# compbio-UofT/shrimp

Measured on AMD Instinct MI355X. Metric: reads/sec mapped (whole node), 100bp LS reads vs 3Gbp ref, 1/2/4/8 GPUs, higher is better.
Workload: dtype int16

## Files before the change

shrimp_amd/csrc/gm_common.h:

```cpp
#pragma once
#include <hip/hip_runtime.h>
#include <stdint.h>
#include <string>
#include <vector>
#include "../../include/gmapper_hip.h"

#define GM_MAX_SEEDS 16
#define GM_WAVE 64

void gm_set_error(const char* fmt, ...);
#define GM_HIP(call)                                                                          \
  do {                                                                                        \
    hipError_t e_ = (call);                                                                   \
    if (e_ != hipSuccess) {                                                                   \
      gm_set_error("%s failed: %s (%s:%d)", #call, hipGetErrorString(e_), __FILE__, __LINE__); \
      return GM_E_NODEVICE;                                                                   \
    }                                                                                         \
  } while (0)

struct GmSeedDev {
  uint64_t mask;
  int span, weight;
  const uint32_t* dir;
  const uint32_t* pos;
  const uint32_t* bkt;
  const uint32_t* sdir;
  const uint32_t* spos;
  uint32_t n_pos;
};

#define GM_MP_CAP 8192
#define GM_MP_FLAG 0x80000000u
struct GmMpDev {
  int mode;
  int dmin[2], dmax[2];
  int mate_dmin[2], mate_dmax[2];
  uint32_t* rows; const uint32_t* cnt;
  uint32_t* out_rows; uint32_t* out_cnt;
};
__device__ __forceinline__ bool gm_mp_reach(const uint32_t* row, uint32_t n, long long lo, long long hi, uint32_t* first = nullptr) {
  if (hi < 0 || n == 0) return false;
  if (lo < 0) lo = 0;
  uint32_t a = 0, z = n;
  while (a < z) { const uint32_t m = (a + z) >> 1; if ((long long)(row[m] & ~GM_MP_FLAG) < lo) a = m + 1; else z = m; }
  if (first) *first = a;
  return a < n && (long long)(row[a] & ~GM_MP_FLAG) <= hi;
}

struct GmIndexDev {
  const uint32_t* genome;
  const uint32_t* genome_cs;
  int colour;
  int hflag;
  int cs_flip;
  int no_region_counts;
  GmMpDev mp;
  const uint8_t* contig_rna;
  int genome_is_rna;
  const uint8_t* read_rna;
  uint64_t total_len;
  int n_contigs;
  const uint32_t* contig_off;
  int n_seeds, min_seed_span, max_seed_span;
  int slab_bits, n_slabs;
  int region_bits, region_overlap;
  uint32_t list_cutoff;
  GmSeedDev seed[GM_MAX_SEEDS];
};

struct GmScoreDev {
  int match, mismatch;
  int a_go, a_ge, b_go, b_ge;
  int anchor_width;
  int match_mode, min_matches;
  int skip_strands;
  int num_tmp_outputs;
  int tiebreak_rev;
  int hash_filter_calls;
  int gapless;
  int local;
  double wgen_thr_frac;
  double vect_thr_frac, full_thr_frac;
  int wgen_abs, vect_abs, full_abs;
};

struct GmHit {
  uint32_t g_off;
  int32_t  ax, ay;
  int32_t  alen, awidth;
  int32_t  score_window_gen;
  int32_t  score_vector;
  int32_t  pct_score_vector;
  uint16_t cn, w_len;
  uint16_t matches, flags;
};

#define GM_MAX_OPS 2048
struct GmFullRes {
  int32_t read_idx;
  int16_t st, gen_st;
  uint32_t cn; uint32_t g_off;
  int32_t w_len;
  int32_t score_vector;
  int32_t score_max, matches, score_window_gen;
  int32_t score;
  int32_t read_start, rmapped, genome_start, gmapped;
  int32_t n_match, n_mismatch, n_ins, n_del;
  int32_t n_ops; uint32_t ops_off;
  int32_t sort_idx;
  uint32_t hit_slot;
  int32_t n_xover;
};

__host__ __device__ __forceinline__ uint64_t gm_cmpl_tab(bool rna) { return 0xFBCDE56879A00123ull + (rna ? 1ull : 0ull); }

#ifdef GM_NO_READ_RNA
#define GM_READ_RNA(ix, rd) false
#else
#define GM_READ_RNA(ix, rd) ((ix).read_rna && (ix).read_rna[rd])
#endif
#define GM_SEAM_RNA 0x100

__device__ __forceinline__ uint32_t gm_read_code(const uint32_t* __restrict__ rw, int read_len, int st, int colour, int i, bool rna = false) {
  if (colour) {
    if (st && i == 0) return 15u;
    const int src = st ? (read_len - i) : i;
    return (rw[src >> 3] >> ((src & 7) * 4)) & 0xf;
  }
  const int src = st ? (read_len - 1 - i) : i;
  uint32_t c = (rw[src >> 3] >> ((src & 7) * 4)) & 0xf;
  if (st) { const uint64_t cm = gm_cmpl_tab(rna); c = (uint32_t)(cm >> (c * 4)) & 0xf; }
  return c;
}

#define GM_HASH_TABLE_POWER 12
__host__ __device__ __forceinline__ uint32_t gm_hash32(uint32_t a) {
  a = (a + 0x7ed55d16u) + (a << 12); a = (a ^ 0xc761c23cu) ^ (a >> 19); a = (a + 0x165667b1u) + (a << 5);
  a = (a + 0xd3a2646cu) ^ (a << 9); a = (a + 0xfd7046c5u) + (a << 3); a = (a ^ 0xb55a4f09u) ^ (a >> 16);
  return a;
}
__device__ __forceinline__ uint32_t gm_mapidx(const GmIndexDev& ix, uint64_t mask, int span, const uint8_t* kmer) {
  uint32_t mapidx = 0;
  if (!ix.hflag) {
    for (int t = 0; t < span; t++) if ((mask >> t) & 1) mapidx = (mapidx << 2) | (kmer[span - 1 - t] & 3u);
    return mapidx;
  }
  const int nw = (ix.max_seed_span + 7) >> 3;
  for (int w = 0; w < nw; w++) {
    uint32_t word = 0;
    for (int t = 0; t < 8; t++) { const int age = 8 * w + t; if (age < span && ((mask >> age) & 1)) word |= (uint32_t)(kmer[span - 1 - age] & 0xfu) << (4 * t); }
    mapidx = gm_hash32(word ^ mapidx);
  }
  return mapidx & ((1u << (2 * GM_HASH_TABLE_POWER)) - 1u);
}

static inline int gm_ceil_div(long long a, long long b) { return (int)((a + b - 1) / b); }
```

shrimp_amd/csrc/gm_host.hip:

```cpp
#include <algorithm>
#include <atomic>
#include <chrono>
#include <cmath>
#include <cstdarg>
#include <cstddef>
#include <cstdio>
#include <cstdlib>
#include <cstring>
#include <memory>
#include <thread>
#include <mutex>
#include <condition_variable>
#include <deque>
#include <functional>
#include <future>
#include <map>
#include <unordered_map>
#include <zlib.h>
#include "gm_common.h"
#include "gm_internal.h"

static thread_local char g_err[512] = "";
void gm_set_error(const char* fmt, ...) {
  va_list ap; va_start(ap, fmt); vsnprintf(g_err, sizeof g_err, fmt, ap); va_end(ap);
}
extern "C" const char* gm_last_error(void) { return g_err; }
extern "C" int gm_device_count(void) { int n = 0; if (hipGetDeviceCount(&n) != hipSuccess) return 0; return n; }
hipError_t gm_lds_at_least(const void* kernel, size_t bytes) {
  if (bytes <= 48 * 1024) return hipSuccess;
  int dev = 0; hipError_t e = hipGetDevice(&dev);
  if (e != hipSuccess) return e;
  static std::mutex m; static std::map<std::pair<int, const void*>, size_t> raised;
  std::lock_guard<std::mutex> lk(m);
  size_t& cur = raised[{dev, kernel}];
  if (bytes <= cur) return hipSuccess;
  e = hipFuncSetAttribute(kernel, hipFuncAttributeMaxDynamicSharedMemorySize, (int)bytes);
  if (e == hipSuccess) cur = bytes;
  return e;
}
static struct { std::mutex m; char* p = nullptr; size_t cap = 0; char* live = nullptr; size_t live_cap = 0; } g_outcache;
static char* outcache_take(size_t want, size_t* cap) {
  std::lock_guard<std::mutex> g(g_outcache.m);
  if (g_outcache.p && g_outcache.cap >= want) { char* r = g_outcache.p; *cap = g_outcache.cap; g_outcache.p = nullptr; g_outcache.cap = 0; return r; }
  return nullptr;
}
static void outcache_track(char* p, size_t cap) { std::lock_guard<std::mutex> g(g_outcache.m); g_outcache.live = p; g_outcache.live_cap = cap; }
static void gm_text_pool_drop();
extern "C" void gm_release_cache(void) { { std::lock_guard<std::mutex> g(g_outcache.m); free(g_outcache.p); g_outcache.p = nullptr; g_outcache.cap = 0; } gm_text_pool_drop(); }
extern "C" void gm_free(void* p) {
  if (!p) return;
  { std::lock_guard<std::mutex> g(g_outcache.m);
    if (p == g_outcache.live && g_outcache.live_cap >= ((size_t)16 << 20)) {
      g_outcache.live = nullptr;
      if (g_outcache.p && g_outcache.cap >= g_outcache.live_cap) {  }
      else { free(g_outcache.p); g_outcache.p = (char*)p; g_outcache.cap = g_outcache.live_cap; return; }
    } else if (p == g_outcache.live) g_outcache.live = nullptr;
  }
  free(p);
}

extern "C" void gm_params_default(gm_params_t* p) {
  memset(p, 0, sizeof *p);
  p->match_score = 10; p->mismatch_score = -15;
  p->a_gap_open_score = -33; p->a_gap_extend_score = -7; p->b_gap_open_score = -33; p->b_gap_extend_score = -3;
  p->window_len = 140.0; p->window_overlap = 90.0; p->window_gen_threshold = 55.0;
  p->sw_vect_threshold = 50.0; p->sw_full_threshold = 50.0;
  p->match_mode = 2; p->num_outputs = 10; p->num_tmp_outputs = 30; p->anchor_width = 8;
  p->region_bits = 11; p->region_overlap = 50; p->list_cutoff = 0; p->hash_filter_calls = 1; p->tiebreak_rev = 1;
  p->sam_unaligned = 0; p->longest_read_len = 1000; p->strata = 0; p->max_alignments = 0;
  p->colour_space = 0; p->crossover_score = -20; p->indel_taboo_len = 0; p->pr_xover = 0.03; p->local_alignment = 0; p->ungapped = 0; p->hash_seeds = 0; p->output_format = 0; p->print_read_seq = 0; p->strand_only = 0;
  p->single_best_mapping = 0; p->all_contigs = 0; p->no_mapping_qualities = 0; p->no_improper_mappings = 0;
  p->extra_sam_fields = 0; p->sam_r2 = 0; memset(p->read_group, 0, sizeof p->read_group);
  p->trim_front = 0; p->trim_end = 0; p->trim_first = 1; p->trim_second = 1; p->trim_illumina = 0; p->min_avg_qv = 10; p->ignore_qvs = 0; p->no_qv_check = 0;
}
extern "C" int gm_abi_sizeof(int which) {
  switch (which) { case 0: return (int)sizeof(gm_params_t); case 1: return (int)sizeof(gm_pair_opts_t); case 2: return (int)sizeof(gm_map_stats_t); case 3: return (int)sizeof(gm_merge_options_t); }
  return -1;
}
static inline bool gm_mqv_on(const gm_params_t& P) { return !P.local_alignment && !P.no_mapping_qualities; }
extern "C" void gm_params_default_cs(gm_params_t* p) {
  gm_params_default(p);
  p->colour_space = 1; p->mismatch_score = -24; p->sw_vect_threshold = 47.0; p->sw_full_threshold = 50.0;
}

static GmScoreDev make_score(const gm_params_t& P) {
  GmScoreDev s; memset(&s, 0, sizeof s);
  s.match = P.match_score;
  s.mismatch = P.colour_space ? P.match_score + P.crossover_score : P.mismatch_score;
  s.a_go = -P.a_gap_open_score; s.a_ge = -P.a_gap_extend_score; s.b_go = -P.b_gap_open_score; s.b_ge = -P.b_gap_extend_score;
  s.anchor_width = P.anchor_width; s.match_mode = P.match_mode; s.min_matches = P.match_mode;
  s.skip_strands = P.strand_only == 1 ? 2 : (P.strand_only == 2 ? 1 : 0);
  s.num_tmp_outputs = P.num_tmp_outputs; s.tiebreak_rev = P.tiebreak_rev; s.hash_filter_calls = P.hash_filter_calls; s.local = P.local_alignment ? 1 : 0; s.gapless = P.ungapped ? 1 : 0;
  auto frac = [](double thr, double* f, int* a) { if (thr < 0) { *f = -1.0; *a = (int)(-thr); } else { *f = thr / 100.0; *a = 0; } };
  frac(P.window_gen_threshold, &s.wgen_thr_frac, &s.wgen_abs);
  frac(P.sw_vect_threshold, &s.vect_thr_frac, &s.vect_abs);
  frac(P.sw_full_threshold, &s.full_thr_frac, &s.full_abs);
  return s;
}

GmIndexDev GmIndexHost::dev_view() const {
  GmIndexDev d; memset(&d, 0, sizeof d);
  d.genome = d_genome; d.genome_cs = d_genome_cs; d.colour = params.colour_space ? 1 : 0; d.hflag = params.hash_seeds ? 1 : 0; d.total_len = total_len; d.n_contigs = n_contigs; d.contig_off = d_contig_off;
  d.contig_rna = d_contig_rna; d.genome_is_rna = genome_is_rna; d.read_rna = nullptr;
  d.n_seeds = n_seeds; d.min_seed_span = min_seed_span; d.max_seed_span = max_seed_span;
  d.slab_bits = slab_bits; d.n_slabs = n_slabs; d.region_bits = params.region_bits; d.region_overlap = params.region_overlap;
  d.list_cutoff = list_cutoff;
  for (int i = 0; i < n_seeds; i++) {
    d.seed[i].mask = seeds[i].mask; d.seed[i].span = seeds[i].span; d.seed[i].weight = seeds[i].weight;
    d.seed[i].dir = seeds[i].d_dir; d.seed[i].pos = seeds[i].d_pos; d.seed[i].bkt = seeds[i].d_bkt; d.seed[i].n_pos = seeds[i].n_pos;
    d.seed[i].sdir = strips_ready ? seeds[i].d_sdir : nullptr; d.seed[i].spos = strips_ready ? seeds[i].d_spos : nullptr;
  }
  return d;
}

static int add_seed(GmIndexHost* ix, const char* s) {
  if (ix->n_seeds >= GM_MAX_SEEDS) return GM_E_ARG;
  GmSeedHost& sd = ix->seeds[ix->n_seeds];
  sd.mask = 0; sd.span = (int)strlen(s); sd.weight = 0; sd.text = s;
  if (sd.span < 1 || sd.span > 32) return GM_E_ARG;
  for (int i = 0; i < sd.span; i++) {
    if (s[i] != '0' && s[i] != '1') return GM_E_ARG;
    sd.mask = (sd.mask << 1) | (uint64_t)(s[i] == '1'); sd.weight += (s[i] == '1');
  }
  if (sd.weight < 1 || (!ix->params.hash_seeds && sd.weight > 14)) return GM_E_ARG;
  sd.kbits = ix->params.hash_seeds ? 2 * GM_HASH_TABLE_POWER : 2 * sd.weight;
  ix->max_seed_span = std::max(ix->max_seed_span, sd.span);
  ix->min_seed_span = std::min(ix->min_seed_span, sd.span);
  ix->n_seeds++;
  return GM_OK;
}

static void choose_slabs(GmIndexHost* ix) {
  int bits = 12;
  while ((1ull << bits) < ix->total_len) bits++;
  int sb = std::min(bits, 29);
  if (const char* e = gm_tune("GM_SLAB_BITS")) sb = std::max(ix->params.region_bits + 2, std::min(31, atoi(e)));
  ix->slab_bits = sb;
  ix->n_slabs = (int)((ix->total_len + (1ull << sb) - 1) >> sb);
  if (ix->n_slabs < 1) ix->n_slabs = 1;
}

static int index_tables(gm_index* ix, int n_contigs, const uint32_t* contig_len, const char* const* contig_names) {
  ix->n_contigs = n_contigs;
  ix->contig_off.resize(n_contigs + 1);
  uint64_t tot = 0;
  for (int c = 0; c < n_contigs; c++) {
    ix->contig_off[c] = (uint32_t)tot; tot += contig_len[c];
    char nm[64]; snprintf(nm, sizeof nm, "contig%d", c + 1);
    ix->names.push_back(contig_names && contig_names[c] ? contig_names[c] : nm);
  }
  if (tot >= (1ull << 32)) { gm_set_error("genome of %llu bp exceeds the reference's 32-bit global coordinates", (unsigned long long)tot); return GM_E_ARG; }
  ix->contig_off[n_contigs] = (uint32_t)tot;
  ix->total_len = tot;
  if (ix->params.list_cutoff == 0) {
    int maxw = 0; for (int i = 0; i < ix->n_seeds; i++) maxw = std::max(maxw, ix->seeds[i].weight);
    if (ix->params.hash_seeds) maxw = GM_HASH_TABLE_POWER;
    uint32_t cutoff = 1000; unsigned long long p4 = 1ull << (2 * maxw);
    if ((uint32_t)((100ull * tot) / p4) > cutoff) cutoff = (uint32_t)((100ull * tot) / p4);
    ix->list_cutoff = cutoff;
  } else ix->list_cutoff = ix->params.list_cutoff;
  choose_slabs(ix);
  ix->genome_words = (tot + 7) / 8 + 64;
  GM_HIP(hipMalloc(&ix->d_contig_off, (size_t)(n_contigs + 1) * 4));
  GM_HIP(hipMemcpy(ix->d_contig_off, ix->contig_off.data(), (size_t)(n_contigs + 1) * 4, hipMemcpyHostToDevice));
  return GM_OK;
}
static int index_prepare(gm_index* ix, int n_contigs, const uint32_t* const* contigs, const uint32_t* contig_len, const char* const* contig_names) {
  { const int rc = index_tables(ix, n_contigs, contig_len, contig_names); if (rc != GM_OK) return rc; }
  std::vector<uint32_t> g(ix->genome_words, 0);
  for (int c = 0; c < n_contigs; c++) {
    const uint64_t off = ix->contig_off[c]; const uint32_t* src = contigs[c]; const uint64_t len = contig_len[c];
    const int sh = (int)(off & 7) * 4; uint64_t w0 = off >> 3; const uint64_t nw = (len + 7) / 8;
    for (uint64_t k = 0; k < nw; k++) {
      uint32_t w = src[k];
      if (k == nw - 1 && (len & 7)) w &= (1u << ((len & 7) * 4)) - 1u;
      g[w0 + k] |= w << sh;
      if (sh) g[w0 + k + 1] |= w >> (32 - sh);
    }
  }
  GM_HIP(hipMalloc(&ix->d_genome, ix->genome_words * 4));
  GM_HIP(hipMemcpy(ix->d_genome, g.data(), ix->genome_words * 4, hipMemcpyHostToDevice));
  return GM_OK;
}

extern "C" void gm_index_free(gm_index_t* ix);
static int index_seeds(gm_index* ix, int n_seeds, const char* const* seeds) {
  int rc = GM_OK;
  if (n_seeds == 0) {
    rc |= add_seed(ix, "11110111101111"); rc |= add_seed(ix, "1111011100100001111"); rc |= add_seed(ix, "1111000011001101111");
  } else for (int i = 0; i < n_seeds; i++) rc |= add_seed(ix, seeds[i]);
  return rc;
}
extern "C" int gm_index_build(gm_index_t** out, int device, int n_contigs, const uint32_t* const* contigs,
                              const uint32_t* contig_len, const char* const* contig_names,
                              int n_seeds, const char* const* seeds, const gm_params_t* params) {
  if (!out || n_contigs < 1 || !contigs || !contig_len) { gm_set_error("gm_index_build: bad arguments"); return GM_E_ARG; }
  if (gm_device_count() <= device) { gm_set_error("no HIP device %d (the seed index lives in HBM; there is no CPU path)", device); return GM_E_NODEVICE; }
  GM_HIP(hipSetDevice(device));
  gm_index* ix = new gm_index();
  ix->device = device;
  if (params) ix->params = *params; else gm_params_default(&ix->params);
  int rc = index_seeds(ix, n_seeds, seeds);
  if (rc != GM_OK) { delete ix; gm_set_error("invalid spaced seed"); return GM_E_ARG; }
  rc = index_prepare(ix, n_contigs, contigs, contig_len, contig_names);
  if (rc != GM_OK) { gm_index_free(ix); return rc; }
  hipStream_t stream; GM_HIP(hipStreamCreate(&stream));
  rc = gm_index_build_device(ix, stream);
  (void)hipStreamDestroy(stream);
  if (rc != GM_OK) { gm_index_free(ix); return rc; }
  *out = ix;
  return GM_OK;
}

extern "C" int gm_index_build_fasta(gm_index_t** out, int device, int n_files, const char* const* paths,
                                    int n_seeds, const char* const* seeds, const gm_params_t* params) {
  if (!out || n_files < 1 || !paths) { gm_set_error("gm_index_build_fasta: bad arguments"); return GM_E_ARG; }
  if (gm_device_count() <= device) { gm_set_error("no HIP device %d (the seed index lives in HBM; there is no CPU path)", device); return GM_E_NODEVICE; }
  GM_HIP(hipSetDevice(device));
  const auto t0 = std::chrono::steady_clock::now();
  gm_index* ix = new gm_index();
  ix->device = device;
  if (params) ix->params = *params; else gm_params_default(&ix->params);
  int rc = index_seeds(ix, n_seeds, seeds);
  if (rc != GM_OK) { delete ix; gm_set_error("invalid spaced seed"); return GM_E_ARG; }
  GmFastaGenome G;
  rc = gm_fasta_to_device(n_files, paths, &G);
  if (rc != GM_OK) { delete ix; return rc; }
  ix->d_genome = G.d_genome;
  std::vector<const char*> nptr(G.names.size());
  for (size_t c = 0; c < G.names.size(); c++) nptr[c] = G.names[c].c_str();
  rc = index_tables(ix, (int)G.lens.size(), G.lens.data(), nptr.data());
  if (rc == GM_OK && (ix->total_len != G.total || ix->genome_words != G.words)) { gm_set_error("gm_index_build_fasta: contig lengths do not add up to the bases packed"); rc = GM_E_ARG; }
  if (rc != GM_OK) { gm_index_free(ix); return rc; }
  const auto t1 = std::chrono::steady_clock::now();
  hipStream_t stream = nullptr;
  if (hipStreamCreate(&stream) != hipSuccess) { gm_index_free(ix); gm_set_error("hipStreamCreate failed"); return GM_E_NODEVICE; }
  rc = gm_index_build_device(ix, stream);
  (void)hipStreamDestroy(stream);
  if (rc != GM_OK) { gm_index_free(ix); return rc; }
  ix->fasta_to_bitfield_s = std::chrono::duration<double>(t1 - t0).count();
  ix->fasta_total_s = std::chrono::duration<double>(std::chrono::steady_clock::now() - t0).count();
  *out = ix;
  return GM_OK;
}
extern "C" int gm_index_n_contigs(const gm_index_t* ix) { return ix ? ix->n_contigs : GM_E_ARG; }
extern "C" int gm_index_contig(const gm_index_t* ix, int c, const char** name, uint32_t* len) {
  if (!ix || c < 0 || c >= ix->n_contigs) { gm_set_error("gm_index_contig: no contig %d", c); return GM_E_ARG; }
  if (name) *name = ix->names[c].c_str();
  if (len) *len = ix->contig_off[c + 1] - ix->contig_off[c];
  return GM_OK;
}
extern "C" int gm_sam_header(const gm_index_t* ix, const char* rg_id, const char* rg_sample, const char* command_line, char** text, size_t* len) {
  if (!ix || !text || !len) { gm_set_error("gm_sam_header: bad arguments"); return GM_E_ARG; }
  std::string h = "@HD\tVN:1.0\tSO:unsorted\n";
  for (int c = 0; c < ix->n_contigs; c++) h += "@SQ\tSN:" + ix->names[c] + "\tLN:" + std::to_string(ix->contig_off[c + 1] - ix->contig_off[c]) + "\n";
  if (rg_id) h += std::string("@RG\tID:") + rg_id + "\tSM:" + (rg_sample ? rg_sample : "") + "\n";
  if (command_line) h += std::string("@PG\tID:gmapper\tVN:2.2.3\tCL:") + command_line + "\n";
  char* p = (char*)malloc(h.size() + 1);
  if (!p) return GM_E_NOMEM;
  memcpy(p, h.c_str(), h.size() + 1);
  *text = p; *len = h.size();
  return GM_OK;
}
extern "C" int gm_index_build_timing(const gm_index_t* ix, double* to_bitfield_s, double* total_s) {
  if (!ix || ix->fasta_total_s <= 0) { gm_set_error("gm_index_build_timing: not an index built by gm_index_build_fasta"); return GM_E_ARG; }
  if (to_bitfield_s) *to_bitfield_s = ix->fasta_to_bitfield_s;
  if (total_s) *total_s = ix->fasta_total_s;
  return GM_OK;
}

extern "C" void gm_index_free(gm_index_t* ix) {
  if (!ix) return;
  (void)hipSetDevice(ix->device);
  (void)hipFree(ix->d_genome); (void)hipFree(ix->d_genome_cs); (void)hipFree(ix->d_contig_off); (void)hipFree(ix->d_contig_rna);
  for (int i = 0; i < ix->n_seeds; i++) { (void)hipFree(ix->seeds[i].d_dir); (void)hipFree(ix->seeds[i].d_pos); (void)hipFree(ix->seeds[i].d_bkt);
                                           (void)hipFree(ix->seeds[i].d_sdir); (void)hipFree(ix->seeds[i].d_spos); }
  delete ix;
}
extern "C" uint32_t gm_index_list_cutoff(const gm_index_t* ix) { return ix->list_cutoff; }
extern "C" int gm_index_n_slabs(const gm_index_t* ix) { return ix->n_slabs; }
extern "C" int gm_index_has_buckets(const gm_index_t* ix) { return ix->seeds[0].d_bkt != nullptr; }
extern "C" uint64_t gm_index_bytes(const gm_index_t* ix) {
  uint64_t b = ix->genome_words * 4 * (ix->d_genome_cs ? 2 : 1);
  for (int i = 0; i < ix->n_seeds; i++) b += (ix->seeds[i].dir_words + (uint64_t)ix->seeds[i].n_pos + (ix->seeds[i].d_bkt ? (16ull << ix->seeds[i].kbits) : 0ull) +
                                            (ix->seeds[i].d_sdir ? (1ull << ix->seeds[i].kbits) + 1 + ix->seeds[i].n_spos : 0ull)) * 4;
  return b;
}
extern "C" int gm_index_get_list(const gm_index_t* ix, int sn, uint32_t mapidx, uint32_t* len, uint32_t* positions, uint32_t cap) {
  if (sn < 0 || sn >= ix->n_seeds || mapidx >= (1u << ix->seeds[sn].kbits)) return GM_E_ARG;
  GM_HIP(hipSetDevice(ix->device));
  uint32_t be[2];
  GM_HIP(hipMemcpy(&be[0], ix->seeds[sn].d_dir + (size_t)mapidx * ix->n_slabs, 4, hipMemcpyDeviceToHost));
  GM_HIP(hipMemcpy(&be[1], ix->seeds[sn].d_dir + (size_t)(mapidx + 1) * ix->n_slabs, 4, hipMemcpyDeviceToHost));
  *len = be[1] - be[0];
  uint32_t n = std::min(*len, cap);
  if (n && positions) GM_HIP(hipMemcpy(positions, ix->seeds[sn].d_pos + be[0], (size_t)n * 4, hipMemcpyDeviceToHost));
  return GM_OK;
}
extern "C" int gm_index_device_array(const gm_index_t* ix, int kind, void** dev_ptr, uint64_t* bytes) {
  if (kind == 0) { *dev_ptr = ix->d_genome; *bytes = ix->genome_words * 4; return GM_OK; }
  if (kind == 1 + 3 * ix->n_seeds) { *dev_ptr = ix->d_genome_cs; *bytes = ix->d_genome_cs ? ix->genome_words * 4 : 0; return GM_OK; }
  const int sn = (kind - 1) / 3, what = (kind - 1) % 3; if (kind < 0 || sn < 0 || sn >= ix->n_seeds) return GM_E_ARG;
  if (what == 0) { *dev_ptr = ix->seeds[sn].d_dir; *bytes = (ix->seeds[sn].dir_words + 16) * 4; }
  else if (what == 1) { *dev_ptr = ix->seeds[sn].d_pos; *bytes = ((uint64_t)ix->seeds[sn].n_pos + 64) * 4; }
  else { *dev_ptr = ix->seeds[sn].d_bkt; *bytes = ix->seeds[sn].d_bkt ? (16ull << ix->seeds[sn].kbits) * 4 : 0; }
  return GM_OK;
}

struct MetaHdr { uint64_t magic, total_len, genome_words; int32_t n_contigs, n_seeds, slab_bits, n_slabs; uint32_t list_cutoff, pad; gm_params_t params;
                 uint32_t n_pos[GM_MAX_SEEDS]; uint64_t dir_words[GM_MAX_SEEDS]; uint32_t has_bkt[GM_MAX_SEEDS]; };
extern "C" int gm_index_meta(const gm_index_t* ix, void* meta, uint64_t* meta_bytes) {
  std::string blob;
  MetaHdr h; memset(&h, 0, sizeof h);
  h.magic = 0x474D4958ull; h.total_len = ix->total_len; h.genome_words = ix->genome_words; h.n_contigs = ix->n_contigs; h.n_seeds = ix->n_seeds;
  h.slab_bits = ix->slab_bits; h.n_slabs = ix->n_slabs; h.list_cutoff = ix->list_cutoff; h.params = ix->params;
  for (int i = 0; i < ix->n_seeds; i++) { h.n_pos[i] = ix->seeds[i].n_pos; h.dir_words[i] = ix->seeds[i].dir_words; h.has_bkt[i] = ix->seeds[i].d_bkt != nullptr; }
  blob.append((const char*)&h, sizeof h);
  blob.append((const char*)ix->contig_off.data(), (size_t)(ix->n_contigs + 1) * 4);
  for (auto& n : ix->names) { blob += n; blob.push_back('\0'); }
  for (int i = 0; i < ix->n_seeds; i++) { blob += ix->seeds[i].text; blob.push_back('\0'); }
  if (meta && *meta_bytes >= blob.size()) memcpy(meta, blob.data(), blob.size());
  *meta_bytes = blob.size();
  return GM_OK;
}
extern "C" int gm_index_alloc_like(gm_index_t** out, int device, const void* meta, uint64_t meta_bytes) {
  if (meta_bytes < sizeof(MetaHdr)) return GM_E_ARG;
  MetaHdr h; memcpy(&h, meta, sizeof h);
  if (h.magic != 0x474D4958ull) return GM_E_ARG;
  if (gm_device_count() <= device) { gm_set_error("no HIP device %d", device); return GM_E_NODEVICE; }
  GM_HIP(hipSetDevice(device));
  gm_index* ix = new gm_index();
  ix->device = device; ix->params = h.params; ix->total_len = h.total_len; ix->genome_words = h.genome_words; ix->n_contigs = h.n_contigs;
  ix->slab_bits = h.slab_bits; ix->n_slabs = h.n_slabs; ix->list_cutoff = h.list_cutoff;
  const char* p = (const char*)meta + sizeof h;
  ix->contig_off.assign((const uint32_t*)p, (const uint32_t*)p + h.n_contigs + 1); p += (size_t)(h.n_contigs + 1) * 4;
  for (int c = 0; c < h.n_contigs; c++) { ix->names.push_back(p); p += strlen(p) + 1; }
  for (int i = 0; i < h.n_seeds; i++) { if (add_seed(ix, p) != GM_OK) { delete ix; return GM_E_ARG; } p += strlen(p) + 1; }
  GM_HIP(hipMalloc(&ix->d_genome, ix->genome_words * 4));
  if (ix->params.colour_space) GM_HIP(hipMalloc(&ix->d_genome_cs, ix->genome_words * 4));
  GM_HIP(hipMalloc(&ix->d_contig_off, (size_t)(h.n_contigs + 1) * 4));
  GM_HIP(hipMemcpy(ix->d_contig_off, ix->contig_off.data(), (size_t)(h.n_contigs + 1) * 4, hipMemcpyHostToDevice));
  for (int i = 0; i < h.n_seeds; i++) {
    ix->seeds[i].n_pos = h.n_pos[i]; ix->seeds[i].dir_words = h.dir_words[i];
    GM_HIP(hipMalloc(&ix->seeds[i].d_dir, (h.dir_words[i] + 16) * 4));
    GM_HIP(hipMalloc(&ix->seeds[i].d_pos, ((uint64_t)h.n_pos[i] + 64) * 4));
    if (h.has_bkt[i]) GM_HIP(hipMalloc(&ix->seeds[i].d_bkt, (16ull << ix->seeds[i].kbits) * 4));
  }
  *out = ix;
  return GM_OK;
}

struct DevSet {
  int cur_len = -1, scap = 0, scap2 = 0, hcap = 0, rcap_per_read = 8, ops_stride = 0, eff_batch = 0;
  int post_threads = 0;
  int p2_grid = 0;
  int8_t* d_xover = nullptr; bool xover_on = false;
  uint8_t* d_qv = nullptr; uint8_t* d_post_bq = nullptr;
  uint8_t* d_read_rna = nullptr;
  uint32_t* d_reads = nullptr; uint8_t* d_initbp = nullptr; uint64_t* d_surv = nullptr; uint32_t* d_surv_cnt = nullptr;
  uint32_t* d_surv_seg = nullptr;
  uint64_t* d_surv2 = nullptr; uint32_t* d_surv_cnt2 = nullptr;
  GmHit* d_hits = nullptr; uint16_t* d_perm = nullptr; uint32_t* d_hit_cnt = nullptr; unsigned long long* d_slots = nullptr;
  uint32_t* d_heavy_list = nullptr; uint32_t* d_heavy_cnt = nullptr;
  int32_t* d_sel = nullptr; int32_t* d_sel_sidx = nullptr; uint32_t* d_sel_cnt = nullptr; uint32_t* d_sel_off = nullptr; uint32_t* d_work = nullptr; uint32_t* d_n_work = nullptr; uint32_t* d_p2_order = nullptr; uint32_t* d_p2_cls = nullptr;
  GmFullRes* d_res = nullptr; uint8_t* d_ops = nullptr; uint8_t* d_back = nullptr; size_t back_stride = 0;
  GmPostRes* d_post = nullptr; double* d_post_fw = nullptr; uint32_t* d_post_info = nullptr;
  int32_t* d_pmin = nullptr; int32_t* d_pmax = nullptr; uint8_t* d_saved = nullptr; uint32_t* d_saved_list = nullptr;
  int caps_pair_mode = 0;
  uint32_t* d_mp_rows = nullptr; uint32_t* d_mp_cnt = nullptr; int mp_rows_for = 0;
};

struct HostSlot {
  GmFullRes* res = nullptr; uint8_t* ops = nullptr; uint32_t* sel_cnt = nullptr; uint32_t* sel_off = nullptr; uint32_t* reads = nullptr;
  uint8_t* post_bq = nullptr; size_t post_bq_cap = 0; bool post_bq_on = false;
  GmPostRes* post = nullptr; size_t post_cap = 0; bool post_on = false;
  size_t res_cap = 0, ops_cap = 0, n_cap = 0, reads_cap = 0; uint32_t n_work = 0;
  bool want_reads = false;
  unsigned long long* stats = nullptr; size_t stats_cap = 0;
};
static int slot_reserve(void** p, size_t* cap, size_t bytes) {
  if (bytes <= *cap) return GM_OK;
  if (*p) (void)hipHostFree(*p);
  *p = nullptr; *cap = 0;
  const size_t want = bytes + bytes / 4 + 4096;
  GM_HIP(hipHostMalloc(p, want, hipHostMallocDefault));
  *cap = want;
  return GM_OK;
}
static void slot_free(HostSlot& h) {
  void* ptrs[] = {h.res, h.ops, h.sel_cnt, h.sel_off, h.reads, h.post, h.post_bq, h.stats};
  for (void* p : ptrs) if (p) (void)hipHostFree(p);
  h = HostSlot();
}

template <class T> struct GmPinVec {
  T* p = nullptr; size_t cap = 0, n = 0;
  int resize(size_t k) { n = k; void* q = p; const int rc = slot_reserve(&q, &cap, k * sizeof(T)); p = (T*)q; return rc; }
  T* data() { return p; } const T* data() const { return p; } T& operator[](size_t i) { return p[i]; } const T& operator[](size_t i) const { return p[i]; } size_t size() const { return n; }
  void release() { if (p) (void)hipHostFree(p); p = nullptr; cap = 0; n = 0; }
};
struct gm_session {
  GmPinVec<GmFullRes> pin_res[8]; GmPinVec<uint8_t> pin_ops[8];
  gm_session* twin = nullptr;
  const gm_index* ix = nullptr;
  gm_params_t P; GmScoreDev sc;
  double score_alpha = 0, score_beta = 0;
  double pr_mismatch = .01, pr_del_open = 0, pr_del_extend = 0, pr_ins_open = 0, pr_ins_extend = 0;
  double* d_qtab = nullptr;
  int max_batch = 0, p2_grid = 16384;
  hipStream_t stream = nullptr;
  hipStream_t stream_b = nullptr;
  hipStream_t stream_c = nullptr;
  hipEvent_t ev[12] = {};
  hipEvent_t pev[2][10] = {};
  hipEvent_t pkev[2][4] = {};
  unsigned long long* d_pstats[2] = {nullptr, nullptr};
  uint32_t* h_pin = nullptr;
  uint32_t flag_epoch = 0, front_epoch[2] = {0, 0}; int front_flag_grid[2] = {0, 0};
  GmK1Scratch k1;
  DevSet set[2];
  DevSet set2[2];
  HostSlot slot[3];
  uint32_t* d_pairs = nullptr; uint32_t* d_pair_cnt = nullptr; int pairs_cap = 0;
  unsigned long long* d_stats = nullptr;
  std::vector<uint32_t> h_genome;
  double last_lookup_ms = 0; uint64_t last_lookup_bytes = 0; int last_lookup_launches = 0;
};

static void free_buffers(DevSet& D) {
  void* ptrs[] = {D.d_read_rna, D.d_xover, D.d_reads, D.d_initbp, D.d_surv, D.d_surv_cnt, D.d_surv_seg, D.d_surv2, D.d_surv_cnt2, D.d_hits, D.d_perm, D.d_hit_cnt, D.d_slots, D.d_heavy_list, D.d_heavy_cnt,
                  D.d_sel, D.d_sel_sidx, D.d_sel_cnt, D.d_sel_off, D.d_work, D.d_n_work, D.d_p2_order, D.d_p2_cls, D.d_res, D.d_ops, D.d_back,
                  D.d_pmin, D.d_pmax, D.d_saved, D.d_saved_list, D.d_post, D.d_post_fw, D.d_post_info, D.d_qv, D.d_post_bq, D.d_mp_rows, D.d_mp_cnt};
  for (void* p : ptrs) if (p) (void)hipFree(p);
  D.d_post = nullptr; D.d_post_fw = nullptr; D.d_post_info = nullptr; D.d_qv = nullptr; D.d_post_bq = nullptr;
  D.d_read_rna = nullptr; D.d_xover = nullptr; D.d_reads = nullptr; D.d_initbp = nullptr; D.d_surv = nullptr; D.d_surv_cnt = nullptr; D.d_surv_seg = nullptr; D.d_surv2 = nullptr; D.d_surv_cnt2 = nullptr; D.d_hits = nullptr; D.d_perm = nullptr; D.d_hit_cnt = nullptr; D.d_slots = nullptr;
  D.d_heavy_list = nullptr; D.d_heavy_cnt = nullptr; D.d_sel = nullptr; D.d_sel_sidx = nullptr; D.d_sel_cnt = nullptr; D.d_sel_off = nullptr;
  D.d_work = nullptr; D.d_n_work = nullptr; D.d_p2_order = nullptr; D.d_p2_cls = nullptr; D.d_res = nullptr; D.d_ops = nullptr; D.d_back = nullptr;
  D.d_pmin = nullptr; D.d_pmax = nullptr; D.d_saved = nullptr; D.d_saved_list = nullptr;
  D.d_mp_rows = nullptr; D.d_mp_cnt = nullptr; D.mp_rows_for = 0;
  D.cur_len = -1;
}

static int pow2ceil(long long v) { int p = 1; while (p < v) p <<= 1; return p; }
static int gm_usable_cores() {
  static const int cached = [] {
    int n = (int)std::max(1u, std::thread::hardware_concurrency());
    long long quota = -1, period = -1;
    if (FILE* f = fopen("/sys/fs/cgroup/cpu.max", "r")) { char q[64] = ""; if (fscanf(f, "%63s %lld", q, &period) == 2 && strcmp(q, "max") != 0) quota = atoll(q); fclose(f); }
    else {
      if (FILE* g = fopen("/sys/fs/cgroup/cpu/cpu.cfs_quota_us", "r")) { if (fscanf(g, "%lld", &quota) != 1) quota = -1; fclose(g); }
      if (FILE* g = fopen("/sys/fs/cgroup/cpu/cpu.cfs_period_us", "r")) { if (fscanf(g, "%lld", &period) != 1) period = -1; fclose(g); }
    }
    if (quota > 0 && period > 0) n = std::min<long long>(n, std::max<long long>(1, (quota + period - 1) / period));
    return n;
  }();
  return cached;
}
static int gm_host_threads() {
  int n = (int)std::min<unsigned>(32, std::max(1u, std::thread::hardware_concurrency()));
  if (const char* e = getenv("GM_HOST_THREADS")) n = std::max(1, atoi(e));
  (void)&gm_usable_cores;
  return n;
}
namespace {
struct GmThreadPool {
  struct Call { const std::function<void()>* fn = nullptr; int left = 0; std::mutex m; std::condition_variable cv; };
  std::mutex m; std::condition_variable cv; std::deque<std::shared_ptr<Call>> q; std::vector<std::thread> workers; bool stop = false;
  ~GmThreadPool() { { std::lock_guard<std::mutex> lk(m); stop = true; } cv.notify_all(); for (auto& t : workers) if (t.joinable()) t.join(); }
  void loop() {
    for (;;) {
      std::shared_ptr<Call> c;
      { std::unique_lock<std::mutex> lk(m); cv.wait(lk, [&] { return stop || !q.empty(); }); if (q.empty()) return; c = std::move(q.front()); q.pop_front(); }
      (*c->fn)();
      { std::lock_guard<std::mutex> lk(c->m); if (--c->left == 0) c->cv.notify_all(); }
    }
  }
  void run(int n, const std::function<void()>& fn) {
    if (n <= 1) { fn(); return; }
    auto c = std::make_shared<Call>(); c->fn = &fn; c->left = n - 1;
    { std::lock_guard<std::mutex> lk(m);
      while ((int)workers.size() < n - 1) workers.emplace_back([this] { loop(); });
      for (int t = 1; t < n; t++) q.push_back(c); }
    cv.notify_all();
    fn();
    std::unique_lock<std::mutex> lk(c->m); c->cv.wait(lk, [&] { return c->left == 0; });
  }
};
GmThreadPool& gm_pool() { static GmThreadPool* p = new GmThreadPool(); return *p; }
}
static void gm_run_on_threads(int n, const std::function<void()>& fn) { gm_pool().run(n, fn); }
namespace {
struct GmTextPool {
  std::mutex m; std::vector<std::string> free_;
  std::string take() { std::lock_guard<std::mutex> lk(m); if (free_.empty()) return std::string(); std::string t = std::move(free_.back()); free_.pop_back(); t.clear(); return t; }
  void give(std::string&& t) { if (t.capacity() == 0 || t.capacity() > (16u << 20)) return; std::lock_guard<std::mutex> lk(m); if (free_.size() < 512) free_.push_back(std::move(t)); }
  void drop() { std::lock_guard<std::mutex> lk(m); free_.clear(); free_.shrink_to_fit(); }
};
GmTextPool& gm_text_pool() { static GmTextPool* p = new GmTextPool(); return *p; }
}
static void gm_text_pool_drop() { gm_text_pool().drop(); }
template <class F> static void gm_parallel_for(size_t n, size_t grain, F fn) {
  const size_t pieces = (n + grain - 1) / std::max<size_t>(1, grain);
  const int nt = (int)std::min<size_t>((size_t)gm_host_threads(), pieces);
  if (nt <= 1) { if (n) fn((size_t)0, n); return; }
  std::atomic<size_t> next(0);
  gm_run_on_threads(nt, [&]() { for (;;) { const size_t c = next.fetch_add(1); if (c >= pieces) break; fn(c * grain, std::min(n, (c + 1) * grain)); } });
}
static bool gm_fixed_lines(const char* text, size_t n, size_t want) {
  if (!n) return true;
  const size_t len = strlen(text), stride = want + 1;
  if (len != n * stride - 1 && len != n * stride) return false;
  std::atomic<bool> ok(true);
  gm_parallel_for(n, 16384, [&](size_t b, size_t e) {
    for (size_t i = b; i < e; i++) {
      const char* p = text + i * stride;
      if (memchr(p, '\n', want) != nullptr || (i + 1 < n && p[want] != '\n')) { ok = false; return; }
    }
  });
  return ok;
}

static int window_len_of(const gm_params_t& P, int read_len) {
  double w = P.window_len < 0 ? -P.window_len : read_len * (P.window_len / 100.0);
  return (int)(uint16_t)w;
}

static int alloc_buffers(gm_session* s, DevSet& D, int read_len, bool paired = false) {
  free_buffers(D);
  const gm_index* ix = s->ix;
  const int read_words = (read_len + 7) / 8;
  const int W = window_len_of(s->P, read_len);
  const double budget = 16e9;
  const double per_read = 2.0 * ((double)(D.scap + D.scap2) * 8 + (double)D.hcap * (sizeof(GmHit) + 2 + 8)) + (double)D.rcap_per_read * (sizeof(GmFullRes) + read_len + W + 16);
  D.eff_batch = (int)std::max(64.0, std::min((double)s->max_batch, budget / per_read));
  const int B = D.eff_batch, rs = 2 * B;
  (void)ix;
  D.ops_stride = ((read_len + W + 15) / 16) * 16;
  D.back_stride = (((size_t)read_len * W + 255) / 256) * 256;
  if (s->P.colour_space) { D.ops_stride *= 2; D.back_stride *= 12; }
  GM_HIP(hipMalloc(&D.d_reads, (size_t)B * read_words * 4 + 64));
  if (!s->P.colour_space) GM_HIP(hipMalloc(&D.d_read_rna, (size_t)B + 64));
  if (s->P.colour_space) { GM_HIP(hipMalloc(&D.d_initbp, (size_t)B + 64)); GM_HIP(hipMalloc(&D.d_xover, (size_t)B * read_len + 64)); GM_HIP(hipMalloc(&D.d_qv, (size_t)B * read_len + 64)); }
  GM_HIP(hipMalloc(&D.d_surv, (size_t)rs * D.scap * 8));
  GM_HIP(hipMalloc(&D.d_surv_cnt, (size_t)rs * 4));
  if (D.scap2 > 0) {
    GM_HIP(hipMalloc(&D.d_surv2, (size_t)rs * D.scap2 * 8)); GM_HIP(hipMalloc(&D.d_surv_cnt2, (size_t)rs * 4));
    GM_HIP(hipMalloc(&D.d_surv_seg, (size_t)rs * (ix->n_slabs + 1) * 4));
  }
  GM_HIP(hipMalloc(&D.d_hits, (size_t)rs * D.hcap * sizeof(GmHit)));
  GM_HIP(hipMalloc(&D.d_perm, (size_t)rs * D.hcap * 2));
  GM_HIP(hipMalloc(&D.d_hit_cnt, (size_t)rs * 4));
  GM_HIP(hipMalloc(&D.d_slots, (size_t)rs * D.hcap * 8));
  GM_HIP(hipMalloc(&D.d_heavy_list, (size_t)rs * 4));
  GM_HIP(hipMalloc(&D.d_heavy_cnt, 4));
  GM_HIP(hipMalloc(&D.d_sel, (size_t)B * GM_SEL_MAX * 4));
  GM_HIP(hipMalloc(&D.d_sel_cnt, (size_t)B * 4));
  GM_HIP(hipMalloc(&D.d_sel_off, (size_t)B * 4));
  const size_t rcap = (size_t)B * D.rcap_per_read;
  GM_HIP(hipMalloc(&D.d_work, (size_t)B * GM_SEL_MAX * 4));
  GM_HIP(hipMalloc(&D.d_n_work, 4));
  GM_HIP(hipMalloc(&D.d_p2_order, (size_t)B * GM_SEL_MAX * 4)); GM_HIP(hipMalloc(&D.d_p2_cls, 16));
  GM_HIP(hipMalloc(&D.d_res, rcap * sizeof(GmFullRes)));
  GM_HIP(hipMalloc(&D.d_ops, rcap * D.ops_stride));
  if (s->P.colour_space && !getenv("GM_POST_SW_HOST")) {
    GM_HIP(hipMalloc(&D.d_post, rcap * sizeof(GmPostRes)));
    D.post_threads = GM_POST_THREADS;
    while (D.post_threads > 16384 && (size_t)D.post_threads * (size_t)(read_len + 1) * 140 > ((size_t)2 << 30)) D.post_threads /= 2;
    if (const char* e = gm_tune("GM_POST_THREADS")) D.post_threads = std::max(4096, std::min(1 << 20, atoi(e) & ~63));
    GM_HIP(hipMalloc(&D.d_post_fw, (size_t)D.post_threads * (size_t)(read_len + 1) * 17 * 8));
    GM_HIP(hipMalloc(&D.d_post_info, (size_t)D.post_threads * (size_t)(read_len + 1) * 4));
    GM_HIP(hipMalloc(&D.d_post_bq, rcap * (size_t)read_len + 64));
  }
  D.p2_grid = (int)std::max<size_t>(256, std::min<size_t>((size_t)s->p2_grid, ((size_t)2 << 30) / D.back_stride));
  GM_HIP(hipMalloc(&D.d_back, (size_t)D.p2_grid * D.back_stride));
  if (paired) {
    GM_HIP(hipMalloc(&D.d_sel_sidx, (size_t)B * GM_SEL_MAX * 4));
    GM_HIP(hipMalloc(&D.d_pmin, (size_t)rs * D.hcap * 4)); GM_HIP(hipMalloc(&D.d_pmax, (size_t)rs * D.hcap * 4));
    GM_HIP(hipMalloc(&D.d_saved, (size_t)rs * D.hcap)); GM_HIP(hipMalloc(&D.d_saved_list, (size_t)B * GM_SEL_MAX * 4));
  }
  D.cur_len = read_len;
  return GM_OK;
}

static void choose_caps(gm_session* s, DevSet& D, int read_len, int pair_mode = 0) {
  const gm_index* ix = s->ix;
  const int max_n_kmers = std::max(0, read_len - ix->min_seed_span + 1);
  double lists = 0, avg_len = 0;
  for (int i = 0; i < ix->n_seeds; i++) {
    lists += std::max(0, read_len - ix->seeds[i].span + 1);
    avg_len += (double)ix->seeds[i].n_pos / (double)(1ull << ix->seeds[i].kbits) / ix->n_seeds;
  }
  const double entries = lists * avg_len;
  const double region = (double)(1 << ix->params.region_bits) + ix->params.region_overlap;
  double expected = entries * std::min(1.0, entries * region / std::max(1.0, (double)ix->total_len)) + lists;
  if (pair_mode ? pair_mode == 2 : s->P.match_mode == 1) expected = entries + lists;
  D.scap = std::min(16384, std::max(256, pow2ceil((long long)(2.2 * expected) + 128)));
  D.hcap = 64;
  D.scap2 = (s->P.match_mode == 2 && !s->P.ungapped && !gm_tune("GM_NO_PRUNE")) ? std::max(std::min(D.scap, std::max(256, pow2ceil((long long)(1.5 * lists)))), D.scap / 8) : 0;
  if (pair_mode == 2 || pair_mode == 3) { D.scap = std::min(D.scap, 4096); D.scap2 = 0; }
  if (const char* e = gm_tune("GM_SCAP")) D.scap = std::min(16384, std::max(64, pow2ceil(atoi(e))));
  if (const char* e = gm_tune("GM_SCAP2")) { if (D.scap2) D.scap2 = std::min(D.scap, std::max(64, pow2ceil(atoi(e)))); }
  if (const char* e = gm_tune("GM_HCAP")) D.hcap = std::min(32768, std::max(4, pow2ceil(atoi(e))));
  (void)max_n_kmers;
}

extern "C" void gm_session_free(gm_session_t* s);
extern "C" int gm_session_create(gm_session_t** out, const gm_index_t* ix, const gm_params_t* params, int max_batch_reads) {
  if (!out || !ix) return GM_E_ARG;
  GM_HIP(hipSetDevice(ix->device));
  gm_session* s = new gm_session();
  s->ix = ix; s->P = params ? *params : ix->params;
  if (s->P.strand_only < 0 || s->P.strand_only > 2) { delete s; gm_set_error("strand_only %d: 0 (both), 1 (-F) or 2 (-C)", params ? params->strand_only : 0); return GM_E_ARG; }
  if (s->P.match_mode != 1 && s->P.match_mode != 2) { delete s; gm_set_error("match_mode %d: 1 or 2 (ref: gmapper.c:2624; 3 and 4 are paired-mode settings with mate-pair region counts)", s->P.match_mode); return GM_E_ARG; }
  if (s->P.ungapped && !s->P.local_alignment) { delete s; gm_set_error("ungapped mode needs local alignment (ref: gmapper.c:2330-2333)"); return GM_E_ARG; }
  if ((s->P.colour_space != 0) != (ix->params.colour_space != 0)) { delete s; gm_set_error("session and index disagree on colour space"); return GM_E_ARG; }
  s->sc = make_score(s->P);
#define GM_HIP_S(call) do { hipError_t e_ = (call); if (e_ != hipSuccess) { gm_set_error("%s: %s", #call, hipGetErrorString(e_)); gm_session_free(s); return GM_E_NODEVICE; } } while (0)
  if (s->P.colour_space) {
    s->score_alpha = (double)s->P.crossover_score / (log(s->P.pr_xover / 3) / log(2.0));
    s->pr_mismatch = 1.0 / (1.0 + 1.0 / 3.0 * pow(2.0, ((double)s->P.match_score - (double)s->P.mismatch_score) / s->score_alpha));
  } else {
    s->pr_mismatch = .01;
    s->score_alpha = ((double)s->P.match_score - (double)s->P.mismatch_score) / (log((1 - s->pr_mismatch) / (s->pr_mismatch / 3.0)) / log(2.0));
  }
  s->score_beta = (double)s->P.match_score - 2 * s->score_alpha - s->score_alpha * log(1 - s->pr_mismatch) / log(2.0);
  s->pr_del_open = pow(2.0, (double)s->P.a_gap_open_score / s->score_alpha);
  s->pr_ins_open = pow(2.0, (double)s->P.b_gap_open_score / s->score_alpha);
  s->pr_del_extend = pow(2.0, (double)s->P.a_gap_extend_score / s->score_alpha);
  s->pr_ins_extend = pow(2.0, ((double)s->P.b_gap_extend_score - s->score_beta) / s->score_alpha);
  if (s->P.colour_space && !getenv("GM_POST_SW_HOST")) {
    std::vector<double> qt(2 * 251);
    for (int q = 0; q <= 250; q++) {
      double e = q <= 0 ? .99999999 : (q >= 250 ? 1E-25 : pow(10.0, -(double)q / 10.0));
      if (e > .75) e = .75;
      qt[2 * q] = log(1 - e); qt[2 * q + 1] = log(e / 3.0);
    }
    GM_HIP_S(hipMalloc(&s->d_qtab, qt.size() * 8));
    GM_HIP_S(hipMemcpy(s->d_qtab, qt.data(), qt.size() * 8, hipMemcpyHostToDevice));
  }
  s->max_batch = std::max(64, std::min(max_batch_reads > 0 ? max_batch_reads : 131072, 1 << 20));
  if (const char* e = gm_tune("GM_P2_GRID")) s->p2_grid = std::max(64, std::min(65536, atoi(e)));
  { int lo = 0, hi = 0; (void)hipDeviceGetStreamPriorityRange(&lo, &hi);
    if (getenv("GM_STREAM_PRIO_OFF") || hi == lo) { GM_HIP_S(hipStreamCreate(&s->stream)); }
    else GM_HIP_S(hipStreamCreateWithPriority(&s->stream, hipStreamDefault, hi)); }
  GM_HIP_S(hipStreamCreateWithFlags(&s->stream_b, hipStreamNonBlocking));
  GM_HIP_S(hipStreamCreateWithFlags(&s->stream_c, hipStreamNonBlocking));
  for (auto& e : s->ev) GM_HIP_S(hipEventCreate(&e));
  for (auto& row : s->pev) for (auto& e : row) GM_HIP_S(hipEventCreate(&e));
  for (auto& row : s->pkev) for (auto& e : row) GM_HIP_S(hipEventCreate(&e));
  GM_HIP_S(hipMalloc(&s->d_stats, (size_t)GS_STRIPES * GS_STRIDE * 8));
  for (auto& d : s->d_pstats) GM_HIP_S(hipMalloc(&d, (size_t)GS_STRIPES * GS_STRIDE * 8));
  GM_HIP_S(hipHostMalloc((void**)&s->h_pin, (16 + 1024) * 4, hipHostMallocDefault));
  memset(s->h_pin, 0, (16 + 1024) * 4);
  { const int rc = gm_index_derive_rna(const_cast<gm_index*>(ix), s->stream); if (rc) { gm_session_free(s); return rc; } }
  if ((ix->n_slabs > 1 || gm_tune("GM_K1_V5")) && !gm_tune("GM_NO_V5") && ix->params.region_bits >= 9 && ix->params.region_bits <= 16) {
    const int rc = gm_index_derive_strips(const_cast<gm_index*>(ix), s->stream);
    if (rc) { gm_session_free(s); return rc; }
  }
  *out = s;
  return GM_OK;
#undef GM_HIP_S
}
extern "C" void gm_session_free(gm_session_t* s) {
  if (!s) return;
  if (s->twin) { gm_session_free(s->twin); s->twin = nullptr; }
  (void)hipSetDevice(s->ix->device);
  for (auto& v : s->pin_res) v.release();
  for (auto& v : s->pin_ops) v.release();
  free_buffers(s->set[0]); free_buffers(s->set[1]); free_buffers(s->set2[0]); free_buffers(s->set2[1]);
  s->k1.release();
  for (auto& h : s->slot) slot_free(h);
  if (s->d_qtab) (void)hipFree(s->d_qtab);
  if (s->d_pairs) (void)hipFree(s->d_pairs);
  if (s->d_pair_cnt) (void)hipFree(s->d_pair_cnt);
  if (s->d_stats) (void)hipFree(s->d_stats);
  for (auto& d : s->d_pstats) if (d) (void)hipFree(d);
  if (s->h_pin) (void)hipHostFree(s->h_pin);
  for (auto& e : s->ev) if (e) (void)hipEventDestroy(e);
  for (auto& row : s->pev) for (auto& e : row) if (e) (void)hipEventDestroy(e);
  for (auto& row : s->pkev) for (auto& e : row) if (e) (void)hipEventDestroy(e);
  if (s->stream) (void)hipStreamDestroy(s->stream);
  if (s->stream_b) (void)hipStreamDestroy(s->stream_b);
  if (s->stream_c) (void)hipStreamDestroy(s->stream_c);
  delete s;
}

struct FHit {
  const GmFullRes* r; const uint8_t* ops;
  int score_full, pass2_key; double pct_score_full; double posterior; int mqv; double z0, z1;
  bool dev_post = false;
  double z2, z3, pr_top_random, insert_size_denom, pr_missed_mp;
  std::string db, qr, qual; int cs_match = 0, cs_mismatch = 0, cs_xover = 0;
};

static inline char* put_uint(char* p, unsigned long long v) {
  static const char D2[201] = "00010203040506070809101112131415161718192021222324252627282930313233343536373839404142434445464748495051525354555657585960616263646566676869707172737475767778798081828384858687888990919293949596979899";
  if (v < 10) { *p++ = (char)('0' + v); return p; }
  char tmp[24]; int n = 0;
  if (v <= 0xFFFFFFFFull) { uint32_t w = (uint32_t)v; while (w >= 100) { const uint32_t r = w % 100; w /= 100; tmp[n++] = D2[2 * r + 1]; tmp[n++] = D2[2 * r]; } if (w >= 10) { tmp[n++] = D2[2 * w + 1]; tmp[n++] = D2[2 * w]; } else tmp[n++] = (char)('0' + w); }
  else { while (v >= 100) { const unsigned r = (unsigned)(v % 100); v /= 100; tmp[n++] = D2[2 * r + 1]; tmp[n++] = D2[2 * r]; } if (v >= 10) { tmp[n++] = D2[2 * v + 1]; tmp[n++] = D2[2 * v]; } else tmp[n++] = (char)('0' + v); }
  while (n) *p++ = tmp[--n];
  return p;
}
static inline char* put_int(char* p, long long v) { if (v < 0) { *p++ = '-'; return put_uint(p, (unsigned long long)(-v)); } return put_uint(p, (unsigned long long)v); }
static inline char* put_str(char* p, const char* s, size_t n) { memcpy(p, s, n); return p + n; }

static int qv_from_pr_corr(double pr_corr) {
  double pr_err = 1 - pr_corr;
  if (pr_err > .99999999) return 0; else if (pr_err < 1E-25) return 250;
  return (int)(-10.0 * log(pr_err) / log(10.0));
}
static int double_to_neglog(double x) { return (int)((double)1000 * -log(x)); }

static int cmp_gen_start(const FHit* a, const FHit* b) {
  if (a->r->cn != b->r->cn) return (int)a->r->cn - (int)b->r->cn;
  if (a->r->gen_st != b->r->gen_st) return a->r->gen_st - b->r->gen_st;
  return a->r->genome_start - b->r->genome_start;
}
static int cmp_gen_end(const FHit* a, const FHit* b) {
  if (a->r->cn != b->r->cn) return (int)a->r->cn - (int)b->r->cn;
  if (a->r->gen_st != b->r->gen_st) return a->r->gen_st - b->r->gen_st;
  return (-a->r->genome_start - a->r->rmapped + a->r->n_del - a->r->n_ins) - (-b->r->genome_start - b->r->rmapped + b->r->n_del - b->r->n_ins);
}
template <class It, class Less> static inline void gm_small_stable_sort(It b, It e, Less less) {
  const auto n = e - b;
  if (n < 2) return;
  if (n > 24) { std::stable_sort(b, e, less); return; }
  for (It i = b + 1; i != e; ++i) {
    auto x = *i; It j = i;
    while (j != b && less(x, *(j - 1))) { *j = *(j - 1); --j; }
    *j = x;
  }
}
template <class Cmp>
static void dedup_pass(std::vector<FHit*>& v, Cmp cmp) {
  if (v.size() < 2) return;
  gm_small_stable_sort(v.begin(), v.end(), [&](const FHit* a, const FHit* b) { return cmp(a, b) < 0; });
  size_t i = 0, k = 0, n = v.size();
  while (i < n) {
    int mx = v[i]->pass2_key; size_t mi = i, j = i + 1;
    while (j < n && !cmp(v[i], v[j])) { if (v[j]->pass2_key > mx) { mx = v[j]->pass2_key; mi = j; } j++; }
    if (mi != k) v[k] = v[mi];
    k++; i = j;
  }
  v.resize(k);
}

static const char CODE2SEQ[17] = "ACGTNNNNNNNNNNNN";
static inline char seq_from_text(char c) {
  switch (c) { case 'R': case 'Y': case 'S': case 'W': case 'K': case 'M': case 'B': case 'D': case 'H': case 'V': return 'N'; default: return c >= 'a' ? (char)(c - 32) : c; }
}
static inline char rc_char(char c) { switch (c) { case 'A': return 'T'; case 'C': return 'G'; case 'G': return 'C'; case 'T': return 'A'; default: return 'N'; } }

struct CsPostConsts {
  double let_m, let_x, col_m[2], col_x[2];
  double pr_del_open, pr_del_extend, pr_ins_open, pr_ins_extend;
  bool sanger = true; int qoff = 0;
};
static CsPostConsts cs_post_consts_from(double pr_snp, double pr_xover, double pr_del_open, double pr_del_extend, double pr_ins_open, double pr_ins_extend,
                                        bool sanger, int qoff) {
  CsPostConsts c; const double ce[2] = {pr_xover, .75};
  c.let_m = log(1 - pr_snp); c.let_x = log(pr_snp / 3.0);
  for (int k = 0; k < 2; k++) { c.col_m[k] = log(1 - ce[k]); c.col_x[k] = log(ce[k] / 3.0); }
  c.pr_del_open = pr_del_open; c.pr_del_extend = pr_del_extend; c.pr_ins_open = pr_ins_open; c.pr_ins_extend = pr_ins_extend; c.sanger = sanger; c.qoff = qoff;
  return c;
}
static CsPostConsts cs_post_consts(const gm_session* s) {
  return cs_post_consts_from(s->pr_mismatch, s->P.pr_xover, s->pr_del_open, s->pr_del_extend, s->pr_ins_open, s->pr_ins_extend, true, 0);
}
static inline void exp_neg16(const double* in, double* out) {
  uint64_t seen[16]; double val[16]; int ns = 0;
  for (int k = 0; k < 16; k++) {
    uint64_t b; memcpy(&b, &in[k], 8);
    int j = 0; while (j < ns && seen[j] != b) j++;
    if (j == ns) { seen[ns] = b; val[ns] = exp(-1 * in[k]); ns++; }
    out[k] = val[j];
  }
}

static void cs_post_sw(const CsPostConsts& K, const uint32_t* rw, int init_bp, int read_start, FHit& h,
                       const char* qual = nullptr, int qual_delta = 33, bool base_quals = false) {
  struct Col { double prior[16], fw[16], bw[16], fs, bs; int col, base_call; };
  std::string& db = h.db; std::string& qr = h.qr;
  static thread_local std::vector<Col> colbuf;
  if (colbuf.size() < db.size() + 1) colbuf.resize(db.size() + 1);
  Col* cols = colbuf.data(); int len = 0;
  auto colour = [&](int j) { return (int)((rw[j >> 3] >> ((j & 7) * 4)) & 0xf); };
  {
    int start_run = 0, j, min_qv = 10000;
    for (j = 0; j < read_start; j++) {
      const int c = colour(j);
      if (c == 15) { start_run = 15; min_qv = 0; j = read_start; break; }
      start_run ^= c;
      if (qual) min_qv = std::min(min_qv, (int)qual[K.qoff + j]);
    }
    for (size_t i = 0; i < db.size(); i++) {
      if (qr[i] == '-') continue;
      Col& c = cols[len];
      int let = -2;
      if (db[i] != '-') switch (db[i]) { case 'A': case 'a': let = 0; break; case 'C': case 'c': let = 1; break; case 'G': case 'g': let = 2; break;
                                         case 'T': case 't': let = 3; break; default: let = -1; }
      const int cc = colour(j); int which;
      if ((len == 0 && start_run == 15) || cc == 15) { c.col = 0; which = 1; } else { c.col = cc ^ (len == 0 ? start_run : 0); which = 0; }
      double col_m = K.col_m[which], col_x = K.col_x[which];
      if (qual && which == 0) {
        const int qv = (len == 0 ? std::min(min_qv, (int)qual[K.qoff + j]) : (int)qual[K.qoff + j]) - qual_delta;
        double e = qv <= 0 ? .99999999 : (qv >= 250 ? 1E-25 : pow(10.0, -(double)qv / 10.0));
        if (!K.sanger) e /= (1 + e);
        if (e > .75) e = .75;
        col_m = log(1 - e); col_x = log(e / 3.0);
      }
      c.base_call = -1;
      switch (qr[i]) { case 'A': case 'a': c.base_call = 0; break; case 'C': case 'c': c.base_call = 1; break; case 'G': case 'g': c.base_call = 2; break;
                       case 'T': case 't': c.base_call = 3; break; default: break; }
      for (int st = 0; st < 16; st++) {
        const int l = (st >> 2) & 3, r = st & 3; double val = 0;
        if (let != -2) val = val - ((r == let) ? K.let_m : K.let_x);
        val = val - (((l ^ r) == c.col) ? col_m : col_x);
        c.prior[st] = val;
      }
      len++; j++;
    }
  }
  if (len == 0) { h.posterior = 0; return; }
  double total;
  {
    Col& a = cols[0]; a.fs = 999999999;
    for (int j = 0; j < 16; j++) { if (((j >> 2) & 3) == init_bp) { a.fw[j] = a.prior[j]; a.fs = (a.fs < a.fw[j]) ? a.fs : a.fw[j]; } else a.fw[j] = HUGE_VAL; }
    for (int j = 0; j < 16; j++) a.fw[j] -= a.fs;
    for (int i = 1; i < len; i++) {
      Col& c = cols[i]; const Col& p = cols[i - 1];
      double e[16], lg[4];
      exp_neg16(p.fw, e);
      for (int l = 0; l < 4; l++) { double sum = 0; for (int k = l; k < 16; k += 4) sum += e[k]; lg[l] = log(sum); }
      c.fs = 999999999;
      for (int j = 0; j < 16; j++) { c.fw[j] = c.prior[j] - lg[(j >> 2) & 3]; c.fs = (c.fs < c.fw[j]) ? c.fs : c.fw[j]; }
      for (int j = 0; j < 16; j++) c.fw[j] -= c.fs;
      c.fs += p.fs;
    }
    double val = 0;
    for (int j = 0; j < 16; j++) val += exp(-1 * (cols[len - 1].fw[j]));
    total = -log(val) + cols[len - 1].fs;
  }
  {
    Col& z = cols[len - 1]; z.bs = 999999999;
    for (int j = 0; j < 16; j++) { z.bw[j] = 0; z.bs = (z.bs < z.bw[j]) ? z.bs : z.bw[j]; }
    for (int j = 0; j < 16; j++) z.bw[j] -= z.bs;
    for (int i = len - 2; i >= 0; i--) {
      Col& c = cols[i]; const Col& n = cols[i + 1];
      double e[16], nl[4];
      { double a[16]; for (int k = 0; k < 16; k++) a[k] = n.prior[k] + n.bw[k]; exp_neg16(a, e); }
      for (int r = 0; r < 4; r++) { double sum = 0; for (int k = 4 * r; k < 4 * r + 4; k++) sum += e[k]; nl[r] = -log(sum); }
      c.bs = 999999999;
      for (int j = 0; j < 16; j++) { c.bw[j] = nl[j & 3]; c.bs = (c.bs < c.bw[j]) ? c.bs : c.bw[j]; }
      for (int j = 0; j < 16; j++) c.bw[j] -= c.bs;
      c.bs += n.bs;
    }
  }
  {
    int j = 0, prev_base = init_bp; h.cs_match = h.cs_mismatch = h.cs_xover = 0; h.qual.clear();
    for (size_t i = 0; i < qr.size(); i++) {
      if (qr[i] == '-') continue;
      const Col& c = cols[j];
      double post[4] = {0, 0, 0, 0};
      { double a[16], ev[16]; for (int st = 0; st < 16; st++) a[st] = c.fw[st] + c.bw[st] + c.fs + c.bs - total; exp_neg16(a, ev);
        for (int st = 0; st < 16; st++) post[st & 3] += ev[st]; }
      int crt = 0; for (int b = 1; b < 4; b++) if (post[b] > post[crt]) crt = b;
      if (qual || base_quals) {
        int t = c.base_call >= 0 ? qv_from_pr_corr(post[c.base_call]) : 0;
        if (t > 40) t = 40;
        h.qual.push_back((char)(33 + t));
      }
      if ((prev_base ^ crt) == c.col) qr[i] = "ACGT"[crt]; else { qr[i] = "acgt"[crt]; h.cs_xover++; }
      if (db[i] != '-') { if (toupper((unsigned char)db[i]) == toupper((unsigned char)qr[i])) h.cs_match++; else h.cs_mismatch++; }
      prev_base = crt; j++;
    }
  }
  {
    double res = exp(-total);
    for (size_t i = 0; i < db.size(); i++) {
      if (db[i] == '-') { res *= K.pr_ins_extend; if (i == 0 || db[i - 1] != '-') res *= K.pr_ins_open; }
      else if (qr[i] == '-') { res *= K.pr_del_extend; if (i == 0 || qr[i - 1] != '-') res *= K.pr_del_open; }
    }
    h.posterior = res;
  }
}
static void cs_alignment_strings(const uint8_t* bt, const uint8_t* codes, int n, std::string& db, std::string& qr, bool recalled = false) {
  static const char L[17] = "ACGTUMRWSYKVHDBN";
  db.clear(); qr.clear();
  for (int t = 0; t < n; t++) {
    const int type = bt[t] & 0x0f; const bool xov = recalled ? (bt[t] & 0x40) != 0 : (bt[t] & 0x80) != 0;
    if (type == 1) { db.push_back(L[codes[t] >> 4]); qr.push_back('-'); continue; }
    char q = recalled ? L[(bt[t] >> 4) & 3] : L[codes[t] & 15]; if (xov) q = (char)tolower((unsigned char)q);
    if (type >= 2 && type <= 5) { db.push_back('-'); qr.push_back(q); continue; }
    const char d = L[codes[t] >> 4];
    if (q == 'n' || q == 'N') q = xov ? (char)tolower((unsigned char)d) : d;
    db.push_back(d); qr.push_back(q);
  }
}

#ifdef GM_HOST_PROFILE
#include <x86intrin.h>
struct GmHpSlots { unsigned long long v[8] = {0, 0, 0, 0, 0, 0, 0, 0}; };
static std::mutex g_hp_m; static std::vector<GmHpSlots*> g_hp_all;
static GmHpSlots& gm_hp_mine() {
  static thread_local GmHpSlots* mine = nullptr;
  if (!mine) { mine = new GmHpSlots(); std::lock_guard<std::mutex> lk(g_hp_m); g_hp_all.push_back(mine); }
  return *mine;
}
struct GmHp { unsigned long long t; GmHpSlots& S; GmHp() : t(__rdtsc()), S(gm_hp_mine()) {} void lap(int k) { const unsigned long long n = __rdtsc(); S.v[k] += n - t; t = n; } };
extern "C" void gm_host_profile_dump(void) {
  static const char* nm[8] = {"post_sw / FHit build", "dedup + sort", "mapping qualities", "record text", "unaligned record", "reads (count)", "", ""};
  unsigned long long g[8] = {0, 0, 0, 0, 0, 0, 0, 0};
  { std::lock_guard<std::mutex> lk(g_hp_m); for (GmHpSlots* s : g_hp_all) for (int k = 0; k < 8; k++) { g[k] += s->v[k]; s->v[k] = 0; } }
  unsigned long long tot = 0; for (int k = 0; k < 5; k++) tot += g[k];
  for (int k = 0; k < 6; k++) { fprintf(stderr, "[host profile] %-22s %14llu%s %5.1f %%\n", nm[k], g[k], k < 5 ? " cycles" : "       ", k < 5 ? 100.0 * g[k] / (tot ? tot : 1) : 0.0); }
  if (g[5]) fprintf(stderr, "[host profile] %.0f cycles per read\n", (double)tot / (double)g[5]);
}
#define GM_HP_DECL GmHp hp_
#define GM_HP(k) hp_.lap(k)
#else
#define GM_HP_DECL do { } while (0)
#define GM_HP(k) do { } while (0)
#endif
struct Finalizer {
  const gm_session* s; int read_len, read_words; const uint32_t* reads;
  const char* const* name_ptr; const int* name_len; long name_base;
  const uint8_t* initbp = nullptr; int ops_half = 0; CsPostConsts csk = CsPostConsts();
  const GmFullRes* res_base = nullptr; const GmPostRes* post_base = nullptr;
  const uint8_t* bq_base = nullptr;
  const char* const* seq_ptr = nullptr;
  const char* const* qual_ptr = nullptr; int qual_delta = 33;
  const uint32_t* hgen = nullptr;

  void ls_alignment_strings(const GmFullRes& r, const uint8_t* ops, int nops, const uint32_t* rw, std::string& db, std::string& qr) const {
    static const char L[17] = "ACGTUMRWSYKVHDBN";
    const gm_index* ix = s->ix; const uint64_t base = ix->contig_off[r.cn]; const int glen = (int)(ix->contig_off[r.cn + 1] - ix->contig_off[r.cn]);
    auto gcode = [&](int j) -> int {
      const uint64_t p = base + (uint64_t)(r.gen_st ? glen - 1 - j : j); int c = (int)((hgen[p >> 3] >> ((p & 7) * 4)) & 0xf);
      if (r.gen_st) c = (int)((0xFBCDE56879A00123ull >> (c * 4)) & 0xf);
      return c; };
    db.clear(); qr.clear();
    int gi = r.genome_start, ri = r.read_start;
    for (int k = 0; k < nops; k++) {
      const char op = (char)ops[k];
      if (op == 'M') { db.push_back(L[gcode(gi++)]); qr.push_back(L[(rw[ri >> 3] >> ((ri & 7) * 4)) & 0xf]); ri++; }
      else if (op == 'I') { db.push_back(L[gcode(gi++)]); qr.push_back('-'); }
      else { db.push_back('-'); qr.push_back(L[(rw[ri >> 3] >> ((ri & 7) * 4)) & 0xf]); ri++; }
    }
  }
  static void edit_string(const std::string& db, const std::string& qr, std::string& o) {
    const int len = (int)db.size(); int consec = 0; bool refgap = false; char nb[16];
    for (int i = 0; i <= len; i++) {
      if (i != len && db[i] == qr[i] && db[i] != '-') { consec++; continue; }
      if (refgap && (consec != 0 || (i == len ? '\0' : db[i]) != '-')) { o += ')'; refgap = false; }
      if (consec != 0) { o.append(nb, snprintf(nb, sizeof nb, "%d", consec)); consec = 0; }
      if (i == len) break;
      if (db[i] == '-') { if (islower((unsigned char)qr[i])) o += 'x'; if (!refgap) o += '('; o += (char)toupper((unsigned char)qr[i]); refgap = true; continue; }
      if (qr[i] == '-') o += '-';
      else if (db[i] == toupper((unsigned char)qr[i])) { o += 'x'; consec++; }
      else if (islower((unsigned char)qr[i])) { o += 'x'; o += (char)toupper((unsigned char)qr[i]); }
// ... 1248 lines not shown
```

shrimp_amd/csrc/gm_internal.h:

```cpp
#pragma once
#include "gm_common.h"

struct GmSeedHost {
  uint64_t mask = 0; int span = 0, weight = 0;
  int kbits = 0;
  uint32_t* d_dir = nullptr; uint32_t* d_pos = nullptr; uint32_t* d_bkt = nullptr;
  uint32_t* d_sdir = nullptr; uint32_t* d_spos = nullptr; uint32_t n_spos = 0;
  uint32_t n_pos = 0; uint64_t dir_words = 0;
  std::string text;
};

struct GmIndexHost {
  int device = 0;
  uint64_t total_len = 0;
  int n_contigs = 0;
  std::vector<uint32_t> contig_off;
  std::vector<std::string> names;
  uint32_t* d_genome = nullptr; uint64_t genome_words = 0;
  uint32_t* d_genome_cs = nullptr;
  uint32_t* d_contig_off = nullptr;
  bool rna_ready = false; std::vector<uint8_t> contig_rna; uint8_t* d_contig_rna = nullptr; int genome_is_rna = 0;
  int n_seeds = 0, min_seed_span = 64, max_seed_span = 0;
  GmSeedHost seeds[GM_MAX_SEEDS];
  int slab_bits = 29, n_slabs = 1;
  gm_params_t params;
  uint32_t list_cutoff = 0;
  bool strips_ready = false;
  double fasta_to_bitfield_s = 0, fasta_total_s = 0;
  GmIndexDev dev_view() const;
};
struct gm_index : GmIndexHost {};

enum { GS_LOOKUPS = 0, GS_ENTRIES, GS_SURVIVORS, GS_ANCHORS, GS_WINDOWS, GS_VEC_CALLS, GS_VEC_CELLS, GS_VEC_BYPASSED,
       GS_FULL_CALLS, GS_FULL_CELLS, GS_EXACT_ORDER, GS_OVERFLOW_SURV, GS_OVERFLOW_HITS, GS_PRUNED, GS_MP_UNFILTERED, GS_N };
#define GS_STRIPES 1024
#define GS_STRIDE 16
#define GS_ADD(stats, slot, val) atomicAdd(&(stats)[(size_t)(blockIdx.x & (GS_STRIPES - 1)) * GS_STRIDE + (slot)], (unsigned long long)(val))

#include <cstdlib>
#include <cctype>
#include <string>
#include <vector>
#ifdef GM_TUNING
static inline const char* gm_tune(const char* name) { return getenv(name); }
#define GM_ABL(bits) (ablate & (bits))
#else
static inline const char* gm_tune(const char*) { return nullptr; }
#define GM_ABL(bits) (false)
#endif

int gm_index_build_device(GmIndexHost* ix, hipStream_t stream);
struct GmFastaGenome { uint32_t* d_genome = nullptr; uint64_t words = 0, total = 0; std::vector<std::string> names; std::vector<uint32_t> lens; };
int gm_fasta_to_device(int n_files, const char* const* paths, GmFastaGenome* out);
static inline std::string gm_extract_name(const std::string& line) {
  size_t b = 1, e = line.find('\t', 1); if (e == std::string::npos) e = line.size();
  while (b < e && isspace((unsigned char)line[b])) b++; while (e > b && isspace((unsigned char)line[e - 1])) e--;
  size_t k = b; while (k < e && line[k] != ' ' && line[k] != '\t') k++;
  return line.substr(b, k - b);
}
int gm_index_colour_genome_device(GmIndexHost* ix, hipStream_t stream);
int gm_index_from_lists_device(GmIndexHost* ix, int sn, const uint32_t* lens, const uint32_t* pos, uint32_t total);

hipError_t gm_lds_at_least(const void* kernel, size_t bytes);

struct GmK1Scratch {
  int cus = 0;
  uint64_t* k4_bins = nullptr; size_t k4_words = 0;
  uint32_t* k4_fb = nullptr;
  uint32_t* k5_fb = nullptr; uint32_t* k5_pl = nullptr; int k5_cap = 0;
  uint2* k5_spill = nullptr; size_t k5_spill_n = 0;
  uint32_t* k1b_list = nullptr; int k1b_cap = 0;
  uint32_t* start_flags = nullptr; int flag_cap = 0; uint32_t epoch = 0;
  int flag_grid = 0, rounds = 1, half = 0; const char* kernel = nullptr;
  void release() {
    void* ptrs[] = {k4_bins, k4_fb, k5_fb, k5_pl, k5_spill, k1b_list};
    for (void* p : ptrs) if (p) (void)hipFree(p);
    *this = GmK1Scratch();
  }
};

struct GmFusePrune { uint64_t* d_surv2; uint32_t* d_surv_cnt2; int scap2; int window_len; int e_max; int* fused; };
int gm_launch_lookup(const GmIndexDev& ix, const uint32_t* d_reads, int n_reads, int read_len, int read_words,
                     uint64_t* d_surv, uint32_t* d_surv_cnt, int scap, uint32_t* d_heavy_list, uint32_t* d_heavy_cnt, int heavy_cap,
                     unsigned long long* d_stats, hipStream_t stream, GmK1Scratch* K, uint32_t* d_surv_seg = nullptr,
                     const GmFusePrune* fuse = nullptr);
int gm_index_derive_rna(GmIndexHost* ix, hipStream_t stream);
int gm_index_derive_strips(GmIndexHost* ix, hipStream_t stream);
int gm_lookup5_launch(const GmIndexDev& ix, const uint32_t* d_reads, int n_reads, int read_len, int read_words, int max_n_kmers, int NL,
                      uint64_t* d_out, uint32_t* d_out_cnt, int out_cap, uint32_t* d_surv_cnt, int prune, uint32_t D, int e_max,
                      uint32_t* d_heavy_list, uint32_t* d_heavy_cnt, int heavy_cap, unsigned long long* d_stats, hipStream_t stream, GmK1Scratch* K,
                      uint64_t* d_raw = nullptr, int raw_cap = 0, uint32_t* d_surv_seg = nullptr);
int gm_launch_lookup_redo(const GmIndexDev& ix, const uint32_t* d_reads, int n_reads, int read_len, int read_words,
                          int n_heavy, const uint32_t* d_redo_list, const uint64_t* d_redo_off, uint64_t* d_out,
                          unsigned long long* d_stats, hipStream_t stream);
size_t gm_lookup_lds_bytes(const GmIndexDev& ix, int read_len);

int gm_launch_prune(int n_reads, int read_len, int window_len, int e_max, int n_slabs, int slab_bits, const uint64_t* d_surv, const uint32_t* d_surv_cnt,
                    const uint32_t* d_surv_seg, int scap,
                    uint64_t* d_surv2, uint32_t* d_surv_cnt2, int scap2, uint32_t* d_heavy_list, uint32_t* d_heavy_cnt, int heavy_cap,
                    unsigned long long* d_stats, hipStream_t stream, GmK1Scratch* K,
                    const uint32_t* d_rs_list = nullptr, const uint32_t* d_rs_cnt = nullptr, int rs_cap = 0);

int gm_launch_anchors(const GmIndexDev& ix, const GmScoreDev& sc, int n_reads, int read_len, int window_len,
                      const uint64_t* d_surv, const uint32_t* d_surv_cnt, int scap,
                      GmHit* d_hits, uint16_t* d_perm, uint32_t* d_hit_cnt, int hcap, unsigned long long* d_stats, hipStream_t stream);
int gm_launch_anchors_heavy(const GmIndexDev& ix, const GmScoreDev& sc, int n_reads, int read_len, int window_len,
                            int n_heavy, const uint32_t* d_heavy_list, const uint64_t* d_seg_off, const uint32_t* d_seg_n,
                            const uint32_t* d_seg_begin32, const uint32_t* d_seg_end32, uint64_t total_keys,
                            uint64_t* d_keys_in, uint64_t* d_keys_sorted, uint32_t* d_aux, uint32_t* d_nxt, uint32_t* d_ord,
                            GmHit* d_hits, uint16_t* d_perm, uint32_t* d_hit_cnt, int hcap, unsigned long long* d_stats, hipStream_t stream);

int gm_launch_pass1(const GmIndexDev& ix, const GmScoreDev& sc, const uint32_t* d_reads, int n_reads, int read_len, int read_words,
                    int window_len, int window_overlap_abs, GmHit* d_hits, const uint16_t* d_perm, const uint32_t* d_hit_cnt, int hcap,
                    unsigned long long* d_slots, unsigned long long* d_stats, hipStream_t stream,
                    const int32_t* d_pair_min = nullptr, const uint8_t* d_saved = nullptr,
                    const uint8_t* d_initbp = nullptr,
                    bool early_stop = false);

#define GM_SEL_MAX 64
int gm_launch_select(const GmScoreDev& sc, int n_reads, int read_len, const GmHit* d_hits, const uint16_t* d_perm,
                     const uint32_t* d_hit_cnt, int hcap, int32_t* d_sel, uint32_t* d_sel_cnt, uint32_t* d_sel_off,
                     uint32_t* d_work, uint32_t* d_n_work, hipStream_t stream, const uint8_t* d_saved = nullptr);
int gm_launch_build_work(int n_reads, const uint32_t* d_sel_cnt, uint32_t* d_sel_off, uint32_t* d_work, uint32_t* d_n_work, hipStream_t stream);
int gm_launch_pass2(const GmIndexDev& ix, const GmScoreDev& sc, const uint32_t* d_reads, int n_reads, int read_len, int read_words,
                    int window_len, GmHit* d_hits, const uint16_t* d_perm, int hcap, const int32_t* d_sel, const uint32_t* d_sel_cnt,
                    const uint32_t* d_work, const uint32_t* d_n_work, GmFullRes* d_res, uint8_t* d_ops, int ops_stride,
                    uint8_t* d_back, size_t back_stride, int grid, unsigned long long* d_stats, hipStream_t stream,
                    const int32_t* d_sel_sidx = nullptr, int input_strand = 0, int write_back = 0,
                    uint32_t* d_order = nullptr, uint32_t* d_cls_cnt = nullptr);

struct GmCsPostDev { double let_m, let_x, col_m[2], col_x[2], pr_del_open, pr_del_extend, pr_ins_open, pr_ins_extend;
                     const uint8_t* qv; const double* qtab; uint8_t* bq; };
struct GmPostRes { double posterior; int32_t cs_match, cs_mismatch, cs_xover, valid; };
#define GM_POST_THREADS 131072
int gm_launch_post_sw_cs(const GmCsPostDev& K, const uint32_t* d_reads, const uint8_t* d_initbp, int read_len, int read_words, const GmFullRes* d_res, uint8_t* d_ops,
                         int ops_stride, const uint32_t* d_n_work, uint32_t res_cap, GmPostRes* d_post, double* d_fw, uint32_t* d_info, int threads, hipStream_t stream);
int gm_launch_pass2_cs(const GmIndexDev& ix, const GmScoreDev& sc, const int* cs_params9, const uint32_t* d_reads, const uint8_t* d_initbp, int n_reads,
                       int read_len, int read_words, int window_len, const GmHit* d_hits, int hcap, const int32_t* d_sel, const uint32_t* d_work,
                       const uint32_t* d_n_work, GmFullRes* d_res, uint8_t* d_ops, int ops_stride, uint32_t* d_back, size_t back_words, int grid,
                       unsigned long long* d_stats, hipStream_t stream, const int8_t* d_xover = nullptr,
                       const int32_t* d_sel_sidx = nullptr,
                       uint32_t* d_order = nullptr, uint32_t* d_cls_cnt = nullptr);

int gm_launch_revcomp_reads(uint32_t* d_reads, int n_reads, int read_len, int read_words, hipStream_t stream, const uint8_t* d_read_rna = nullptr);
int gm_launch_read_rna_flags(const uint32_t* d_reads, int n_reads, int read_len, int read_words, uint8_t* d_flags, hipStream_t stream);
struct MpDelta { int amin[2], amax[2], bmin[2], bmax[2]; };
MpDelta gm_mp_region_deltas(int region_bits, const int* dmin1, const int* dmax1, const int* dmin2, const int* dmax2);
int gm_launch_mp_filter(int n_pairs, int region_bits, int region_overlap, uint64_t* d_surv1, uint32_t* d_cnt1, int scap1, uint64_t* d_surv2, uint32_t* d_cnt2, int scap2,
                        const int* dmin1, const int* dmax1, const int* dmin2, const int* dmax2, uint32_t* d_seg1, uint32_t* d_seg2, int n_slabs,
                        unsigned long long* d_unfiltered, hipStream_t stream);
int gm_launch_pair_up(int n_pairs, const GmHit* hits1, const uint16_t* perm1, const uint32_t* cnt1, int hcap1,
                      const GmHit* hits2, const uint16_t* perm2, const uint32_t* cnt2, int hcap2,
                      int32_t* pmin1, int32_t* pmax1, int32_t* pmin2, int32_t* pmax2, const int* delta_min, const int* delta_max, hipStream_t stream);
int gm_launch_pair_select(const GmScoreDev& sc, int n_pairs, int len1, int len2,
                          const GmHit* hits1, const uint16_t* perm1, const uint32_t* cnt1, int hcap1, const int32_t* pmin1, const int32_t* pmax1,
                          const GmHit* hits2, const uint16_t* perm2, const uint32_t* cnt2, int hcap2,
                          int32_t* sel1, int32_t* sidx1, uint32_t* selcnt1, int32_t* sel2, int32_t* sidx2, uint32_t* selcnt2,
                          uint32_t* pairs, uint32_t* pair_cnt, hipStream_t stream);
int gm_launch_mark_saved(uint8_t* d_saved, const uint32_t* d_list, int n, hipStream_t stream);

int gm_launch_sw_vector_batch(const GmScoreDev& sc, int n, const uint32_t* d_genome, const long long* d_goff, const int* d_glen,
                              const uint32_t* d_reads, int read_words, const int* d_rlen, int max_g, int max_r, int* d_scores, hipStream_t stream,
                              int early_thr = 0, uint8_t* d_stopped = nullptr);

int gm_launch_sw_full_single(const GmScoreDev& sc, const uint32_t* d_genome, long long goff, int glen, const uint32_t* d_read, int rlen,
                             long long ax, long long ay, int alen, int awidth, int revcmpl, uint8_t* d_back, int* d_out, uint8_t* d_ops, int ops_cap,
                             hipStream_t stream, int has_anchor = 1, int thresh = 0, int maxscore = 0, int local = 0);

int gm_launch_sw_gapless_batch(int n, int match, int mismatch, const uint32_t* d_genome, const uint32_t* d_genome_ls, const long long* d_woff, const int* d_glen,
                               const uint32_t* d_reads, int read_words, const int* d_rlen, const int* d_gidx, const int* d_ridx, const int* d_initbp, int max_r,
                               int* d_scores, hipStream_t stream);
int gm_launch_sw_vector_batch_cs(const GmScoreDev& sc, int n, const uint32_t* d_genome_cs, const uint32_t* d_genome_ls, const long long* d_goff,
                                 const int* d_glen, const uint32_t* d_reads, int read_words, const int* d_rlen, const int* d_initbp, int max_g, int max_r,
                                 int* d_scores, hipStream_t stream);
int gm_launch_sw_full_cs_single(const int* cs_params9, const uint32_t* d_genome_ls, long long goff, int glen, const uint32_t* d_read, int rlen, int initbp,
                                int thresh, long long ax, long long ay, int alen, int awidth, int revcmpl, uint32_t* d_back, int* d_out, uint8_t* d_ops,
                                int ops_cap, hipStream_t stream, int local = 0, const int8_t* d_xrow = nullptr);
```

shrimp_amd/csrc/gm_lookup5.hip:

```cpp
#include <algorithm>
#include <cmath>
#include <mutex>
#include "gm_common.h"
#include "gm_internal.h"
#include <rocprim/device/device_scan.hpp>

typedef uint32_t k5_u32x4 __attribute__((ext_vector_type(4), aligned(4)));
typedef __attribute__((address_space(3))) uint32_t k5_lds_u32;
#define K5_LDS(off) ((k5_lds_u32*)(uintptr_t)(uint32_t)(off))
typedef __attribute__((address_space(3))) uint16_t k5_lds_u16;
#define K5_LDS16(off) ((k5_lds_u16*)(uintptr_t)(uint32_t)(off))
#define K5_LDS_OR(off, m) __hip_atomic_fetch_or(K5_LDS(off), (m), __ATOMIC_RELAXED, __HIP_MEMORY_SCOPE_WORKGROUP)

#ifndef K5_Q
#define K5_Q 4
#endif
enum { C_NCAND = 0, C_OVERFLOW, C_NMEMB, C_NKEEP, C_NSTRIP, C_NEDGE, C_NLISTS , C_SINK = 8, C_NRAW = 9, C_NDEFER = 10, C_NCAND0 = 11 , C_SPILL = 12 , C_WORDS = 16 };
#define K5_MAX_ROUNDS 4

#ifdef K5_STAMPS
__device__ unsigned long long k5_stamps[16];
#define K5_STAMP(i) do { if (tid == 0) { const unsigned long long t_ = __builtin_amdgcn_s_memtime(); atomicAdd(&k5_stamps[i], t_ - t_prev); t_prev = t_; } } while (0)
extern "C" int gm_debug_k5_stamps(unsigned long long* out) {
  unsigned long long z[16] = {0, 0, 0, 0, 0, 0, 0, 0, 0, 0, 0, 0, 0, 0, 0, 0};
  if (hipMemcpyFromSymbol(out, HIP_SYMBOL(k5_stamps), sizeof z) != hipSuccess) return GM_E_NODEVICE;
  if (hipMemcpyToSymbol(HIP_SYMBOL(k5_stamps), z, sizeof z) != hipSuccess) return GM_E_NODEVICE;
  return GM_OK;
}
#else
#define K5_STAMP(i) do { } while (0)
#endif

struct K5Args {
  const uint32_t* reads; int n_reads, read_len, read_words, max_n_kmers, NL;
  int lsw, ltw;
  int cand_cap, hbits;
  int cand_limit;
  int xrec;
  int rounds; uint32_t round_regs;
  uint2* spill; int spill_cap;
  uint64_t* out; uint32_t* out_cnt; int out_cap; uint32_t* surv_cnt;
  int prune; uint32_t D; int e_max;
  uint32_t* heavy_list; uint32_t* heavy_cnt; int heavy_cap;
  unsigned long long* stats;
  uint32_t* fb_list; uint32_t* fb_cnt; int fb_cap;
  uint32_t* start_flags; uint32_t start_epoch;
  uint64_t* raw_out; int raw_cap; uint32_t* surv_seg; int n_slabs; uint32_t* pl_list; uint32_t* pl_cnt; int pl_cap;
};

__device__ __forceinline__ uint32_t k5_lane_times(int lane, uint32_t W) {
  uint32_t r; asm("v_mul_u32_u24 %0, %1, %2" : "=v"(r) : "v"(lane), "s"(W)); return r;
}

#include "gm_region_table.h"

#define K5_KERNEL_HEAD template <int LSWC> __global__ void __launch_bounds__(1024) k_lookup_v5(GmIndexDev ix, K5Args a)
#define K5_KERNEL_MULTI false
#include "gm_lookup5_kernel.inc"
#undef K5_KERNEL_HEAD
#undef K5_KERNEL_MULTI
#define K5_KERNEL_HEAD __global__ void __launch_bounds__(1024) __attribute__((amdgpu_waves_per_eu(5, 5))) k_lookup_v5_rounds(GmIndexDev ix, K5Args a)
#define K5_KERNEL_MULTI true
#define K5_KERNEL_LSWC 15
#include "gm_lookup5_kernel.inc"
#undef K5_KERNEL_HEAD
#undef K5_KERNEL_MULTI
#undef K5_KERNEL_LSWC
#define K5_KERNEL_HEAD __global__ void __launch_bounds__(1024) __attribute__((amdgpu_waves_per_eu(5, 5))) k_lookup_v5_half(GmIndexDev ix, K5Args a)
#define K5_KERNEL_MULTI true
#define K5_KERNEL_LSWC 14
#define K5_KERNEL_BLOOM true
#include "gm_lookup5_kernel.inc"
#undef K5_KERNEL_HEAD
#undef K5_KERNEL_BLOOM
#ifdef GM_TUNING
#define K5_KERNEL_HEAD __global__ void __launch_bounds__(1024) __attribute__((amdgpu_waves_per_eu(5, 5))) k_lookup_v5_half_plain(GmIndexDev ix, K5Args a)
#define K5_KERNEL_BLOOM false
#include "gm_lookup5_kernel.inc"
#undef K5_KERNEL_HEAD
#undef K5_KERNEL_BLOOM
#endif
#undef K5_KERNEL_MULTI
#undef K5_KERNEL_LSWC

__device__ __forceinline__ bool k5_strip(uint32_t p, int rb, uint32_t ovl) { return (p & ((1u << rb) - 1u)) < ovl && (p >> rb) > 0u; }

__global__ void __launch_bounds__(256) k_strip_count(const uint32_t* __restrict__ pos, uint32_t n_pos, int rb, uint32_t ovl, uint32_t* __restrict__ grp_cnt, uint32_t n_groups) {
  const uint32_t lane = threadIdx.x & 63u;
  uint64_t g = ((uint64_t)blockIdx.x * blockDim.x + threadIdx.x) >> 6;
  const uint64_t stride = ((uint64_t)gridDim.x * blockDim.x) >> 6;
  for (; g < n_groups; g += stride) {
    const uint64_t i = g * 64 + lane;
    const bool f = i < n_pos && k5_strip(pos[i], rb, ovl);
    const unsigned long long b = __ballot(f);
    if (lane == 0) grp_cnt[g] = (uint32_t)__popcll(b);
  }
}
__global__ void __launch_bounds__(256) k_strip_scatter(const uint32_t* __restrict__ pos, uint32_t n_pos, int rb, uint32_t ovl, const uint32_t* __restrict__ grp_rank,
                                                       uint32_t n_groups, uint32_t* __restrict__ spos) {
  const uint32_t lane = threadIdx.x & 63u;
  uint64_t g = ((uint64_t)blockIdx.x * blockDim.x + threadIdx.x) >> 6;
  const uint64_t stride = ((uint64_t)gridDim.x * blockDim.x) >> 6;
  for (; g < n_groups; g += stride) {
    const uint64_t i = g * 64 + lane;
    const uint32_t p = i < n_pos ? pos[i] : 0u;
    const bool f = i < n_pos && k5_strip(p, rb, ovl);
    const unsigned long long b = __ballot(f);
    if (f) spos[grp_rank[g] + (uint32_t)__popcll(b & ((1ull << lane) - 1ull))] = p;
  }
}
__global__ void __launch_bounds__(256) k_strip_dir(const uint32_t* __restrict__ dir, const uint32_t* __restrict__ pos, uint32_t n_pos, uint64_t K, int S, int rb, uint32_t ovl,
                                                   const uint32_t* __restrict__ grp_rank, uint32_t* __restrict__ sdir) {
  uint64_t k = (uint64_t)blockIdx.x * blockDim.x + threadIdx.x;
  const uint64_t stride = (uint64_t)gridDim.x * blockDim.x;
  for (; k <= K; k += stride) {
    const uint32_t i = dir[k * (uint64_t)S];
    uint32_t r = grp_rank[i >> 6];
    for (uint32_t q = i & ~63u; q < i; q++) r += k5_strip(pos[q], rb, ovl) ? 1u : 0u;
    sdir[k] = r;
  }
}

static std::mutex g_strip_mutex;
int gm_index_derive_strips(GmIndexHost* ix, hipStream_t stream) {
  std::lock_guard<std::mutex> lock(g_strip_mutex);
  if (ix->strips_ready) return GM_OK;
  const int rb = ix->params.region_bits; const uint32_t ovl = (uint32_t)ix->params.region_overlap;
  for (int sn = 0; sn < ix->n_seeds; sn++) {
    GmSeedHost& sd = ix->seeds[sn];
    const uint64_t K = 1ull << sd.kbits;
    const uint32_t n_groups = (uint32_t)(((uint64_t)sd.n_pos + 63) / 64) + 1u;
    uint32_t *d_cnt = nullptr, *d_rank = nullptr; void* tmp = nullptr; size_t tmp_bytes = 0;
    GM_HIP(hipMalloc(&d_cnt, (size_t)n_groups * 4)); GM_HIP(hipMalloc(&d_rank, (size_t)n_groups * 4));
    hipLaunchKernelGGL(k_strip_count, dim3(256 * 16), dim3(256), 0, stream, sd.d_pos, sd.n_pos, rb, ovl, d_cnt, n_groups);
    hipError_t e = rocprim::exclusive_scan(nullptr, tmp_bytes, d_cnt, d_rank, 0u, (size_t)n_groups, rocprim::plus<uint32_t>(), stream);
    if (e != hipSuccess) { gm_set_error("exclusive_scan size query: %s", hipGetErrorString(e)); return GM_E_NODEVICE; }
    GM_HIP(hipMalloc(&tmp, tmp_bytes ? tmp_bytes : 16));
    e = rocprim::exclusive_scan(tmp, tmp_bytes, d_cnt, d_rank, 0u, (size_t)n_groups, rocprim::plus<uint32_t>(), stream);
    if (e != hipSuccess) { gm_set_error("exclusive_scan: %s", hipGetErrorString(e)); return GM_E_NODEVICE; }
    uint32_t total = 0;
    GM_HIP(hipMemcpyAsync(&total, d_rank + (n_groups - 1), 4, hipMemcpyDeviceToHost, stream));
    GM_HIP(hipStreamSynchronize(stream));
    sd.n_spos = total;
    GM_HIP(hipMalloc(&sd.d_spos, ((size_t)total + 64) * 4));
    GM_HIP(hipMemsetAsync(sd.d_spos, 0xff, ((size_t)total + 64) * 4, stream));
    GM_HIP(hipMalloc(&sd.d_sdir, (size_t)(K + 1 + 16) * 4));
    hipLaunchKernelGGL(k_strip_scatter, dim3(256 * 16), dim3(256), 0, stream, sd.d_pos, sd.n_pos, rb, ovl, d_rank, n_groups, sd.d_spos);
    hipLaunchKernelGGL(k_strip_dir, dim3(256 * 16), dim3(256), 0, stream, sd.d_dir, sd.d_pos, sd.n_pos, K, ix->n_slabs, rb, ovl, d_rank, sd.d_sdir);
    GM_HIP(hipGetLastError());
    GM_HIP(hipStreamSynchronize(stream));
    (void)hipFree(d_cnt); (void)hipFree(d_rank); (void)hipFree(tmp);
  }
  ix->strips_ready = true;
  return GM_OK;
}

int gm_lookup5_launch(const GmIndexDev& ix, const uint32_t* d_reads, int n_reads, int read_len, int read_words, int max_n_kmers, int NL,
                      uint64_t* d_out, uint32_t* d_out_cnt, int out_cap, uint32_t* d_surv_cnt, int prune, uint32_t D, int e_max,
                      uint32_t* d_heavy_list, uint32_t* d_heavy_cnt, int heavy_cap, unsigned long long* d_stats, hipStream_t stream, GmK1Scratch* K,
                      uint64_t* d_raw, int raw_cap, uint32_t* d_surv_seg) {
  int dev = 0; if (hipGetDevice(&dev) != hipSuccess) return 0;
  if (!ix.seed[0].sdir || ix.region_bits < 9 || ix.region_bits > 16 || NL <= 0) return 0;
  const bool forced = gm_tune("GM_K1_V5") != nullptr;
  double entries = 0;
  for (int sn = 0; sn < ix.n_seeds; sn++) {
    const double lists = std::max(0, read_len - ix.seed[sn].span + 1 - ix.colour);
    entries += lists * (double)ix.seed[sn].n_pos / (double)(1ull << (ix.hflag ? 2 * GM_HASH_TABLE_POWER : 2 * ix.seed[sn].weight));
  }
  if (!forced && entries < 8000.0) return 0;
  const size_t budget = 160 * 1024 - 512;
  const size_t fixed0 = (size_t)24 * NL + 2 * (size_t)((read_len + 15) & ~15) + C_WORDS * 4 + GM_MAX_SEEDS * 32;
  const size_t full_tables = (size_t)(4u << 15) + (size_t)(4u << 12);
  int xrec = read_len > 128 ? 16 : 64;
  if (fixed0 + 24 * (size_t)xrec + full_tables > budget && fixed0 + 24 * 16 + full_tables <= budget) xrec = (int)((budget - full_tables - fixed0) / 24);
  const size_t fixed = fixed0 + 24 * (size_t)xrec;
  int lsw = 15;
  int threads = 1024;
  bool small_shape = false;
  if (!forced && ix.colour && NL <= 512 && !gm_tune("GM_K5_LSW") && !gm_tune("GM_K1_THREADS") && !(gm_tune("GM_K5_SMALL") && atoi(gm_tune("GM_K5_SMALL")) == 0)) {
    const double lam = entries * (double)((1u << ix.region_bits) + ix.region_overlap) / std::max(1.0, (double)ix.total_len);
    const double memb = 2.0 * entries * std::min(1.0, lam), late = 0.5 * entries * std::min(1.0, entries / (double)(32ull << 14));
    const double first = entries * std::min(1.0, (late + 0.5 * memb) / (double)(32ull << 11));
    const double cap14 = (double)(((4u << 14) / 4u / 6u) & ~15u);
    if (memb + late + first <= 0.5 * cap14 && fixed + (size_t)(4u << 14) + (size_t)(4u << 11) <= 96 * 1024) { small_shape = true; lsw = 14; threads = 512; }
  }
  int half = 0;
  if (const char* e = gm_tune("GM_K5_HALF")) half = atoi(e);
  const size_t half_budget = 80 * 1024 - 512, half_tables = (size_t)(4u << 14) + (size_t)(4u << 11);
  if (half && (ix.region_bits < 11 || NL > 512 || fixed0 + 24 * 8 + half_tables > half_budget)) half = 0;
  if (half) { lsw = 14; threads = 512; xrec = (int)std::min<size_t>(64, (half_budget - half_tables - fixed0) / 24); }
  if (half) if (const char* e = gm_tune("GM_K5_HALF_THREADS")) threads = std::max(64, std::min(1024, atoi(e) & ~63));
  const size_t fixed_h = fixed0 + 24 * (size_t)xrec;
  if (!half)
  if (const char* e = gm_tune("GM_K5_LSW")) lsw = std::max(8, std::min(15, atoi(e)));
  while (!half && lsw >= 8 && fixed + (size_t)(4u << lsw) + (size_t)(4u << (lsw - 3)) > budget) lsw--;
  if (lsw < 8) return 0;
  if (!half)
  if (const char* e = gm_tune("GM_K1_THREADS")) { const int v = std::max(64, std::min(1024, atoi(e))); threads = 64; while (threads * 2 <= v) threads *= 2; }
  const int ltw = lsw - 3;
  const int hbits = lsw - 2;
  const int cand_cap = (int)(((4u << lsw) / 4u / 6u) & ~15u);
  if (cand_cap < 16) return 0;
  int cand_limit = cand_cap - 8, rounds = 1;
  if (!forced) {
    const double lam = entries * (double)((1u << ix.region_bits) + ix.region_overlap) / std::max(1.0, (double)ix.total_len);
    const double memb = 2.0 * entries * std::min(1.0, lam), late = 0.5 * entries * std::min(1.0, entries / (double)(32ull << (lsw + (half == 1 ? 1 : 0))));
    const double first = entries * std::min(1.0, (late + 0.5 * memb) / (double)(32ull << (lsw - 3)));
    if (memb + late + first > 0.85 * cand_cap) {
      rounds = (int)std::ceil((memb + late + first) / ((half ? 0.95 : 1.25) * cand_cap));
      rounds = std::max(rounds, 2);
      if (rounds > K5_MAX_ROUNDS || NL > threads || lsw != (half ? 14 : 15)) return 0;
    }
  }
  if (const char* e = gm_tune("GM_K5_ROUNDS")) { rounds = std::max(1, std::min(K5_MAX_ROUNDS, atoi(e))); if (rounds > 1 && (NL > threads || lsw != (half ? 14 : 15))) return 0; }
  const uint32_t n_regs = (uint32_t)((ix.total_len + (1ull << ix.region_bits) - 1) >> ix.region_bits);
  const uint32_t round_regs = std::max(1u, (n_regs + (uint32_t)rounds - 1u) / (uint32_t)rounds);
  if (const char* e = gm_tune("GM_K5_CANDLIMIT")) cand_limit = std::max(1, std::min(cand_limit, atoi(e)));
  if (prune && (D + (uint32_t)std::max(0, e_max) > (1u << ix.region_bits) || D > 0xFFFFu)) return 0;
  const size_t lds = (half ? fixed_h : fixed) + (size_t)(4u << lsw) + (size_t)(4u << ltw);
  const int fb_cap = std::max(4096, 2 * n_reads);
  if (!K->cus) { if (hipDeviceGetAttribute(&K->cus, hipDeviceAttributeMultiprocessorCount, dev) != hipSuccess || K->cus < 1) K->cus = 256; }
  if (fb_cap > K->k5_cap) {
    if (K->k5_fb) { (void)hipStreamSynchronize(stream); (void)hipFree(K->k5_fb); (void)hipFree(K->k5_pl); K->k5_fb = nullptr; K->k5_pl = nullptr; K->k5_cap = 0; }
    if (hipMalloc(&K->k5_fb, (size_t)(fb_cap + 4) * 4) != hipSuccess) return 0;
    if (hipMalloc(&K->k5_pl, (size_t)(fb_cap + 4) * 4) != hipSuccess) return 0;
    K->k5_cap = fb_cap;
  }
  uint32_t* const fb_cnt_p = K->k5_fb + K->k5_cap; uint32_t* const pl_cnt_p = K->k5_pl + K->k5_cap;
  if (hipMemsetAsync(fb_cnt_p, 0, 4, stream) != hipSuccess || hipMemsetAsync(pl_cnt_p, 0, 4, stream) != hipSuccess) return GM_E_NODEVICE;
  if (gm_lds_at_least((const void*)k_lookup_v5<15>, lds) != hipSuccess || gm_lds_at_least((const void*)k_lookup_v5<14>, lds) != hipSuccess ||
      gm_lds_at_least((const void*)k_lookup_v5_rounds, lds) != hipSuccess || gm_lds_at_least((const void*)k_lookup_v5_half, lds) != hipSuccess ||
#ifdef GM_TUNING
      gm_lds_at_least((const void*)k_lookup_v5_half_plain, lds) != hipSuccess ||
#endif
      gm_lds_at_least((const void*)k_lookup_v5<0>, lds) != hipSuccess) return 0;
  int grid = std::min(2 * n_reads, (half || small_shape) ? 2 * K->cus : K->cus);
  if (const char* e = gm_tune("GM_K5_GRID")) grid = std::max(1, std::min(2 * n_reads, atoi(e)));
  K5Args a;
  a.reads = d_reads; a.n_reads = n_reads; a.read_len = read_len; a.read_words = read_words; a.max_n_kmers = max_n_kmers; a.NL = NL;
  a.lsw = lsw; a.ltw = ltw; a.cand_cap = cand_cap; a.hbits = hbits; a.cand_limit = cand_limit; a.xrec = xrec; a.rounds = rounds; a.round_regs = round_regs;
  a.out = d_out; a.out_cnt = d_out_cnt; a.out_cap = out_cap; a.surv_cnt = d_surv_cnt; a.prune = prune; a.D = D; a.e_max = e_max;
  a.heavy_list = d_heavy_list; a.heavy_cnt = d_heavy_cnt; a.heavy_cap = heavy_cap; a.stats = d_stats;
  a.fb_list = K->k5_fb; a.fb_cnt = fb_cnt_p; a.fb_cap = fb_cap;
  a.raw_out = prune ? d_raw : nullptr; a.raw_cap = raw_cap; a.surv_seg = d_surv_seg; a.n_slabs = ix.n_slabs; a.pl_list = K->k5_pl; a.pl_cnt = pl_cnt_p; a.pl_cap = fb_cap;
  a.spill = nullptr; a.spill_cap = cand_cap;
  if (rounds > 1) {
    const size_t need = (size_t)grid * (size_t)(rounds - 1) * (size_t)cand_cap;
    if (need > K->k5_spill_n) {
      if (K->k5_spill) { (void)hipStreamSynchronize(stream); (void)hipFree(K->k5_spill); K->k5_spill = nullptr; K->k5_spill_n = 0; }
      if (hipMalloc(&K->k5_spill, need * sizeof(uint2)) != hipSuccess) return 0;
      K->k5_spill_n = need;
    }
    a.spill = K->k5_spill;
  }
  const bool use_flags = K->start_flags && grid <= K->flag_cap;
  K->flag_grid = use_flags ? grid : 0;
  a.start_flags = use_flags ? K->start_flags : nullptr; a.start_epoch = K->epoch;
  K->rounds = rounds; K->half = half;
  if (half) {
#ifdef GM_TUNING
    if (half == 2) hipLaunchKernelGGL(k_lookup_v5_half_plain, dim3(grid), dim3(threads), lds, stream, ix, a); else
#endif
    hipLaunchKernelGGL(k_lookup_v5_half, dim3(grid), dim3(threads), lds, stream, ix, a);
  } else if (rounds > 1) hipLaunchKernelGGL(k_lookup_v5_rounds, dim3(grid), dim3(threads), lds, stream, ix, a);
  else if (lsw == 15) hipLaunchKernelGGL((k_lookup_v5<15>), dim3(grid), dim3(threads), lds, stream, ix, a);
  else if (lsw == 14) hipLaunchKernelGGL((k_lookup_v5<14>), dim3(grid), dim3(threads), lds, stream, ix, a);
  else hipLaunchKernelGGL((k_lookup_v5<0>), dim3(grid), dim3(threads), lds, stream, ix, a);
  if (hipGetLastError() != hipSuccess) return GM_E_NODEVICE;
  return 1;
}
```

shrimp_amd/csrc/gm_lookup5_kernel.inc:

```
K5_KERNEL_HEAD {
  constexpr bool MULTI = K5_KERNEL_MULTI;
#ifdef K5_KERNEL_BLOOM
  constexpr bool BLOOM = K5_KERNEL_BLOOM;
#else
  constexpr bool BLOOM = false;
#endif
#ifdef K5_KERNEL_LSWC
  constexpr int LSWC = K5_KERNEL_LSWC;
#endif
  if (a.start_flags && threadIdx.x == 0) __hip_atomic_store(&a.start_flags[blockIdx.x], a.start_epoch, __ATOMIC_RELAXED, __HIP_MEMORY_SCOPE_SYSTEM);
  __builtin_amdgcn_s_setprio(3);
  extern __shared__ __align__(16) uint32_t smem[];
  const int tid = threadIdx.x, nthr = blockDim.x, lane = tid & (GM_WAVE - 1);
  const int wv = __builtin_amdgcn_readfirstlane(tid >> 6), nwv = nthr >> 6;
  const int S = ix.n_slabs, rb = ix.region_bits, lsw = LSWC ? LSWC : a.lsw, ltw = lsw - 3, hbits = lsw - 2;
  const int cand_cap = LSWC ? (int)(((4u << LSWC) / 4u / 6u) & ~15u) : a.cand_cap;
  const uint32_t rmask = (1u << rb) - 1u, ovl = (uint32_t)ix.region_overlap;
  const uint32_t wmask = (1u << lsw) - 1u, tmask = (1u << ltw) - 1u;
  if ((uint32_t)(uintptr_t)(k5_lds_u32*)smem != 0u) __builtin_trap();
  uint32_t* twice = smem;
  uint32_t* seen = smem + (1u << ltw);
  uint32_t* candp = seen;
  uint16_t* candy = (uint16_t*)(candp + cand_cap);
  uint32_t* htag = seen + (1u << hbits);
  uint32_t* hmin = htag + (1u << hbits);
  uint32_t* hmax = hmin + (1u << hbits);
  uint32_t* rec = seen + (1u << lsw);
  const int RC = a.NL + a.xrec;
  uint32_t* srec = rec + 4 * RC;
  uint8_t* codes = (uint8_t*)(srec + 2 * RC);
  uint32_t* ctrl = (uint32_t*)(codes + 2 * ((a.read_len + 15) & ~15));
  const uint32_t smask4 = wmask << 2, tmask4 = tmask << 2, swb = 4u << ltw;
  const int sh_a = rb - 2, sh_b = rb + lsw;
  const uint32_t hmask = (1u << hbits) - 1u; const int hshift = 32 - hbits;
  const uint32_t pb_cap = MULTI ? (2u << hbits) : (uint32_t)cand_cap;
  const uint32_t pb_pos = MULTI ? swb + (4u << hbits) : swb, pb_y = pb_pos + 4u * pb_cap;
  uint32_t* const sb_pos = MULTI ? htag : candp; uint16_t* const sb_y = (uint16_t*)(sb_pos + pb_cap);
  const int hclr_q = (int)(3u << hbits) >> 2;
  const int tab_q = (int)(((1u << ltw) + (1u << lsw)) >> 2);
  const uint32_t* __restrict__ pos0 = ix.seed[0].pos;
  const uint32_t* __restrict__ spos0 = ix.seed[0].spos;
  unsigned long long my_lookups = 0, my_entries = 0;
  uint32_t k_prune = __builtin_amdgcn_readfirstlane(a.prune != 0 ? 1u : 0u), k_D = __builtin_amdgcn_readfirstlane(a.D);
  uint32_t k_emax_on = __builtin_amdgcn_readfirstlane(a.e_max >= 0 ? 1u : 0u), k_emax = __builtin_amdgcn_readfirstlane((uint32_t)max(a.e_max, 0));
  asm volatile("" : "+s"(k_prune), "+s"(k_D), "+s"(k_emax_on), "+s"(k_emax));

  { uint4* t4 = (uint4*)smem; for (int w = tid; w < tab_q; w += nthr) t4[w] = make_uint4(0, 0, 0, 0); }
  if (tid < C_WORDS) ctrl[tid] = 0;

  auto bloom_mask = [&](const uint32_t t) -> uint32_t { return (1u << (t & 31u)) | (2u << ((t + (((t >> 5) & 3u) << 2)) & 31u)); };
  auto mark = [&](const uint32_t p) {
    const uint32_t av = p >> sh_a, t = p >> sh_b, m1 = 1u << (t & 31u), m = BLOOM ? bloom_mask(t) : m1;
    const uint32_t old = K5_LDS_OR(swb + (av & smask4), m);
    if ((old & m) == m) K5_LDS_OR(av & tmask4, m1);
  };
  auto has2 = [&](const uint32_t p) -> bool { return (*K5_LDS((p >> sh_a) & tmask4) >> ((p >> sh_b) & 31u)) & 1u; };

#ifdef K5_STAMPS
  unsigned long long t_prev = __builtin_amdgcn_s_memtime();
#endif
  const bool ahead = a.NL <= nthr;
  const uint32_t cpad = (uint32_t)((a.read_len + 15) & ~15);
  uint32_t pf_b = 0, pf_e = 0, pf_sb = 0, pf_se = 0; bool pf_ok = false;
  auto fill_codes = [&](const int r, uint8_t* cb) {
    if (r >= 2 * a.n_reads) return;
    const uint32_t* rw = a.reads + (size_t)(r >> 1) * a.read_words;
    for (int i = tid; i < a.read_len; i += nthr) cb[i] = (uint8_t)gm_read_code(rw, a.read_len, (r & 1) ^ ix.cs_flip, ix.colour, i, GM_READ_RNA(ix, r >> 1));
  };
  uint32_t* stab = ctrl + C_WORDS;
  if (tid < ix.n_seeds) {
    const GmSeedDev& sd = ix.seed[tid];
    const uint64_t d = (uint64_t)(uintptr_t)sd.dir, sdp = (uint64_t)(uintptr_t)sd.sdir, po = (uint64_t)(sd.pos - pos0), so = (uint64_t)(sd.spos - spos0);
    *(uint4*)&stab[8 * tid] = make_uint4((uint32_t)d, (uint32_t)(d >> 32), (uint32_t)sdp, (uint32_t)(sdp >> 32));
    *(uint4*)&stab[8 * tid + 4] = make_uint4((uint32_t)po, (uint32_t)(po >> 32), (uint32_t)so, (uint32_t)(so >> 32));
  }
  int k_sn = 0, k_i = 0, k_span = 0; uint64_t k_mask = 0; bool k_ok = false;
  const int k_stride = 1, k_slot = tid;
  const int nsw = ahead ? min(nwv, (a.NL + GM_WAVE - 1) / GM_WAVE) : nwv;
  if (ahead && k_slot < a.NL) {
    k_sn = k_slot / a.max_n_kmers; k_i = k_slot - k_sn * a.max_n_kmers;
    k_span = ix.seed[k_sn].span; k_mask = ix.seed[k_sn].mask;
    k_ok = k_i >= ix.colour && k_i + k_span <= a.read_len;
    if (!k_ok) { k_span = 0; k_mask = 0; }
  }
  uint32_t* cnl_w = nullptr;
  auto strip_of = [&](const int j0, uint32_t& slen) -> const uint32_t* {
    const uint2 sr = *(const uint2*)&srec[2 * j0];
    const uint4 st = *(const uint4*)&stab[8 * (rec[4 * j0 + 3] & 15u) + 4];
    slen = sr.y;
    return spos0 + ((((uint64_t)st.w << 32) | st.z) + sr.x);
  };
  auto put_records = [&](const uint64_t la, const uint32_t len, const uint32_t ysn, const uint32_t sb, const uint32_t slen) {
    const uint32_t nch = (len + 255u) >> 8;
    const uint32_t j = atomicAdd(cnl_w, nch);
    for (uint32_t c = 0; c < nch && j + c < (uint32_t)RC; c++) {
      const uint64_t ca = la + ((uint64_t)c << 10);
      *(uint4*)&rec[4 * (j + c)] = make_uint4((uint32_t)ca, (uint32_t)(ca >> 32), min(256u, len - (c << 8)), ((ysn >> 12) & 0xFFF0u) | (ysn & 0xFu));
      *(uint2*)&srec[2 * (j + c)] = c ? make_uint2(0u, 0u) : make_uint2(sb, slen);
    }
  };
  auto put_list = [&](const uint32_t b, const uint32_t n, const uint32_t sb, const uint32_t sn) {
    const uint4 so = *(const uint4*)&stab[8 * k_sn + 4];
    const uint64_t ptr = (((uint64_t)so.y << 32) | so.x) + b;
    put_records((uint64_t)(uintptr_t)(pos0 + ptr), n, ((uint32_t)k_i << 16) | (uint32_t)k_sn, sb, sn);
  };
  auto kmer_ahead = [&](const int r, const uint8_t* cb) {
    pf_ok = k_ok && r < 2 * a.n_reads;
    uint32_t mapidx = 0;
    if (wv >= nsw) {}
    else if (!ix.hflag) {
      for (int t0 = 0; t0 < ix.max_seed_span; t0 += 8) {
        uint32_t c[8];
#pragma unroll
        for (int u = 0; u < 8; u++) { const int x = k_i + k_span - 1 - t0 - u; c[u] = cb[min(max(x, 0), a.read_len - 1)]; }
#pragma unroll
        for (int u = 0; u < 8; u++) mapidx = ((k_mask >> (t0 + u)) & 1ull) ? ((mapidx << 2) | (c[u] & 3u)) : mapidx;
      }
    } else if (pf_ok) mapidx = gm_mapidx(ix, k_mask, k_span, cb + k_i);
    if (!pf_ok) mapidx = 0;
    const uint4 sp = *(const uint4*)&stab[8 * k_sn];
    typedef const uint32_t __attribute__((address_space(1)))* k5_gptr;
    const k5_gptr dir = (k5_gptr)(((uint64_t)sp.y << 32) | sp.x) + (size_t)mapidx * (uint32_t)S;
    const k5_gptr sdir = (k5_gptr)(((uint64_t)sp.w << 32) | sp.z) + mapidx;
    pf_b = dir[0]; pf_e = dir[S]; pf_sb = sdir[0]; pf_se = sdir[1];
  };
  uint32_t rf_lo[K5_MAX_ROUNDS], rf_m1[K5_MAX_ROUNDS];
#pragma unroll
  for (int d = 0; d < K5_MAX_ROUNDS; d++) {
    const uint64_t rsz64 = 1ull << rb, lo = (uint64_t)d * a.round_regs * rsz64, hi = d >= a.rounds - 1 ? (1ull << 32) : lo + (uint64_t)a.round_regs * rsz64;
    const uint64_t flo = lo >= rsz64 ? lo - rsz64 : 0ull, fhi = hi + rsz64 < (1ull << 32) ? hi + rsz64 : (1ull << 32);
    rf_lo[d] = (uint32_t)std::min<uint64_t>(flo, 0xFFFFFFFFull); rf_m1[d] = MULTI && d < a.rounds && flo < (1ull << 32) ? (uint32_t)(fhi - 1ull - flo) : 0u;
  }
  uint2* const spill_wg = MULTI ? a.spill + (size_t)blockIdx.x * (size_t)(a.rounds - 1) * a.spill_cap : nullptr;
  __syncthreads();
  if (ahead) { fill_codes(blockIdx.x, codes); __syncthreads(); kmer_ahead(blockIdx.x, codes); }
  int it = 0;
  for (int rs = blockIdx.x; rs < 2 * a.n_reads; rs += gridDim.x, it++) {
    uint32_t* const cnl = &ctrl[C_NLISTS + (it & 1)];
    cnl_w = cnl;
    if (ahead) {
      fill_codes(rs + (int)gridDim.x, codes + (uint32_t)((it + 1) & 1) * cpad);
      const uint32_t b = pf_b, e = pf_e, sb = pf_sb, se = pf_se;
      if ((b ^ e ^ sb ^ se) == 0x9E3779B9u && e - b == 0x7F4A7C15u) ctrl[C_SINK] = 1u;
      const bool has_list = pf_ok && e != b && e - b <= ix.list_cutoff;
      if (pf_ok) my_lookups++;
      if (has_list) { my_entries += (e - b); put_list(b, e - b, sb, se - sb); }
      __syncthreads();
      K5_STAMP(8);
      kmer_ahead(rs + (int)gridDim.x, codes + (uint32_t)((it + 1) & 1) * cpad);
      K5_STAMP(9);
    } else {
    const int rd = rs >> 1, st = rs & 1;
    const uint32_t* rw = a.reads + (size_t)rd * a.read_words;
    for (int i = tid; i < a.read_len; i += nthr) codes[i] = (uint8_t)gm_read_code(rw, a.read_len, st ^ ix.cs_flip, ix.colour, i, GM_READ_RNA(ix, rd));
    __syncthreads();
    for (int off = tid; off < a.NL; off += nthr) {
      const int sn = off / a.max_n_kmers, i = off - sn * a.max_n_kmers;
      const int span = ix.seed[sn].span;
      if (i < ix.colour || i + span > a.read_len) continue;
      const uint32_t mapidx = gm_mapidx(ix, ix.seed[sn].mask, span, codes + i);
      const uint32_t* dir = ix.seed[sn].dir + (size_t)mapidx * (uint32_t)S;
      my_lookups++;
      const uint32_t b = dir[0], e = dir[S];
      if (e == b || e - b > ix.list_cutoff) continue;
      const uint32_t sb = ix.seed[sn].sdir[mapidx], se = ix.seed[sn].sdir[mapidx + 1];
      my_entries += (e - b);
      put_records((uint64_t)(uintptr_t)(ix.seed[sn].pos + b), e - b, ((uint32_t)i << 16) | (uint32_t)sn, sb, se - sb);
    }
    __syncthreads();
    }
    K5_STAMP(0);
    const int nl_raw = (int)*cnl, nl = min(nl_raw, RC);
    const bool rec_over = nl_raw > RC;

    struct Step { uint32_t n, ysn; const uint32_t* src; };
    const int xh = min(nl, nwv - nsw);
    int gj = wv, gnext = wv;
    uint4 gr = make_uint4(0, 0, 0, 0);
    auto gen_reset = [&]() { gnext = xh + wv; gj = (wv >= nsw && wv - nsw < xh) ? wv - nsw : gnext; if (gj == gnext) gnext += nwv; if (gj < nl) gr = *(const uint4*)&rec[4 * gj]; };
    auto gen = [&](Step& s) {
      s.n = 0; s.ysn = 0; s.src = pos0;
      if (gj < nl) {
        const uint64_t o = ((uint64_t)__builtin_amdgcn_readfirstlane(gr.y) << 32) | (uint32_t)__builtin_amdgcn_readfirstlane(gr.x);
        s.n = __builtin_amdgcn_readfirstlane(gr.z); s.ysn = __builtin_amdgcn_readfirstlane(gr.w);
        s.src = (const uint32_t*)(const uint32_t __attribute__((address_space(1)))*)(uintptr_t)o;
        gj = gnext; gnext += nwv; if (gj < nl) gr = *(const uint4*)&rec[4 * gj];
      }
    };
#undef K5_GEN_B
#undef K5_GEN_RESET_B
#ifdef K5_REV_B
    const int g_first = xh + wv, g_ahead = (wv >= nsw && wv - nsw < xh) ? wv - nsw : -1;
    auto gen_reset_rev = [&]() {
      gj = g_first < nl ? g_first + ((nl - 1 - g_first) / nwv) * nwv : g_ahead;
      if (gj >= 0) gr = *(const uint4*)&rec[4 * gj];
    };
    auto gen_rev = [&](Step& s) {
      s.n = 0; s.ysn = 0; s.src = pos0;
      if (gj >= 0) {
        const uint64_t o = ((uint64_t)__builtin_amdgcn_readfirstlane(gr.y) << 32) | (uint32_t)__builtin_amdgcn_readfirstlane(gr.x);
        s.n = __builtin_amdgcn_readfirstlane(gr.z); s.ysn = __builtin_amdgcn_readfirstlane(gr.w);
        s.src = (const uint32_t*)(const uint32_t __attribute__((address_space(1)))*)(uintptr_t)o;
        gj = gj >= g_first ? (gj - nwv >= g_first ? gj - nwv : g_ahead) : -1;
        if (gj >= 0) gr = *(const uint4*)&rec[4 * gj];
      }
    };
#define K5_GEN_B gen_rev
#define K5_GEN_RESET_B gen_reset_rev
#else
#define K5_GEN_B gen
#define K5_GEN_RESET_B gen_reset
#endif
    auto issue = [&](const Step& s, k5_u32x4& v) {
      const uint32_t W = (s.n + 63u) >> 6, x = k5_lane_times(lane, W), lim = max(s.n, 1u) - 1u;
      const uint32_t e = (x < lim ? x : lim) << 2;
#ifdef K5_ASM_LOADS
      asm volatile("global_load_dwordx4 %0, %1, %2" : "=&v"(v) : "v"(e), "s"(s.src) : "memory");
#else
      v = *(const k5_u32x4*)((const char*)s.src + e);
#endif
    };
#ifndef K5_ASM_LOADS
#define K5_WAIT_OLDEST(v) asm volatile("" : "+v"(v))
#elif defined(K5_DEBUG_WAIT0)
#define K5_WAIT_OLDEST(v) asm volatile("s_waitcnt vmcnt(0)" : "+v"(v) :: "memory")
#else
#define K5_WAIT_OLDEST(v) asm volatile("s_waitcnt vmcnt(%1)" : "+v"(v) : "n"(K5_Q - 1) : "memory")
#endif
#ifdef K5_TWICE_BRANCH
#define K5_TWICE(av, t) do { if (t) K5_LDS_OR((av) & tmask4, (t)); } while (0)
#else
#define K5_TWICE(av, t) K5_LDS_OR((av) & tmask4, (t))
#endif

#ifdef K5_ABL_A_TWICE
    for (int a_rep = 0; a_rep < 2; a_rep++)
#endif
    {
#ifndef K5_ABL_NOSTRIP
      for (int j0 = tid >> 2; j0 < nl; j0 += nthr >> 2) {
        uint32_t slen; const uint32_t* sp = strip_of(j0, slen);
        for (uint32_t e = (uint32_t)(tid & 3) * 4u; e < slen; e += 16u) {
          const k5_u32x4 v = *(const k5_u32x4*)(sp + e);
          const uint32_t nv = min(4u, slen - e);
          mark(v.x - (1u << rb));
          if (nv > 1) mark(v.y - (1u << rb));
          if (nv > 2) mark(v.z - (1u << rb));
          if (nv > 3) mark(v.w - (1u << rb));
        }
      }
#endif
      gen_reset();
      Step sd[K5_Q]; k5_u32x4 sv[K5_Q];
#pragma unroll
      for (int q = 0; q < K5_Q; q++) { gen(sd[q]); issue(sd[q], sv[q]); }
      while (sd[0].n) {
#pragma unroll
        for (int q = 0; q < K5_Q; q++) {
          K5_WAIT_OLDEST(sv[q]);
          const uint32_t W = (sd[q].n + 63u) >> 6;
          if (k5_lane_times(lane, W) < sd[q].n) {
            const uint32_t a0 = sv[q].x >> sh_a, a1 = sv[q].y >> sh_a, a2 = sv[q].z >> sh_a, a3 = sv[q].w >> sh_a;
            const uint32_t k1 = W > 1u ? 0xFFFFFFFFu : 0u, k2 = W > 2u ? 0xFFFFFFFFu : 0u;
            const uint32_t t0 = sv[q].x >> sh_b, t1 = sv[q].y >> sh_b, t2 = sv[q].z >> sh_b, t3 = sv[q].w >> sh_b;
            const uint32_t b0 = 1u << (t0 & 31u), b1 = (1u << (t1 & 31u)) & k1, b2 = (1u << (t2 & 31u)) & k2, b3 = 1u << (t3 & 31u);
            const uint32_t m0 = BLOOM ? bloom_mask(t0) : b0, m1 = BLOOM ? bloom_mask(t1) & k1 : b1, m2 = BLOOM ? bloom_mask(t2) & k2 : b2, m3 = BLOOM ? bloom_mask(t3) : b3;
            uint32_t o3 = 0;
#ifdef K5_ABL_A_NOLDS
            const uint32_t sink = (swb + (a0 & smask4)) ^ m0 ^ (swb + (a1 & smask4)) ^ m1 ^ (swb + (a2 & smask4)) ^ m2 ^ a3 ^ m3;
            asm volatile("" :: "v"(sink));
            (void)o3; (void)b0; (void)b1; (void)b2; (void)b3;
#else
            const uint32_t o0 = K5_LDS_OR(swb + (a0 & smask4), m0);
            const uint32_t o1 = K5_LDS_OR(swb + (a1 & smask4), m1);
            const uint32_t o2 = K5_LDS_OR(swb + (a2 & smask4), m2);
            if (W > 3) o3 = K5_LDS_OR(swb + (a3 & smask4), m3);
            if (BLOOM) {
              K5_TWICE(a0, (o0 & m0) == m0 ? b0 : 0u);
              K5_TWICE(a1, (o1 & m1) == m1 ? b1 : 0u);
              K5_TWICE(a2, (o2 & m2) == m2 ? b2 : 0u);
              if (W > 3) K5_TWICE(a3, (o3 & m3) == m3 ? b3 : 0u);
            } else {
            K5_TWICE(a0, o0 & m0);
            K5_TWICE(a1, o1 & m1);
            K5_TWICE(a2, o2 & m2);
            if (W > 3) K5_TWICE(a3, o3 & m3);
            }
#endif
          }
          gen(sd[q]); issue(sd[q], sv[q]);
        }
      }
#ifdef K5_ABL_A_TWICE
      if (a_rep == 0) { __syncthreads(); K5_STAMP(12); }
#endif
    }
    Step sdB[K5_Q]; k5_u32x4 svB[K5_Q];
    K5_GEN_RESET_B();
#pragma unroll
    for (int q = 0; q < K5_Q; q++) { K5_GEN_B(sdB[q]); issue(sdB[q], svB[q]); }
    __syncthreads();
    K5_STAMP(1);
    bool fallback = false;
    uint32_t nc = 0;
    const int nrounds = MULTI ? a.rounds : 1;
      {
      if (!MULTI) { uint4* h4 = (uint4*)htag; for (int w = tid; w < hclr_q; w += nthr) h4[w] = make_uint4(0, 0, 0, 0); }
      {
        for (int j0 = tid >> 2; j0 <
#ifdef K5_ABL_NOSTRIP
             0
#else
             nl
#endif
             ; j0 += nthr >> 2) {
          uint32_t slen; const uint32_t* sp = strip_of(j0, slen);
          const uint32_t ysn = rec[4 * j0 + 3];
          for (uint32_t e = (uint32_t)(tid & 3) * 4u; e < slen; e += 16u) {
            const k5_u32x4 v = *(const k5_u32x4*)(sp + e);
            const uint32_t nv = min(4u, slen - e);
            const bool a0 = !has2(v.x) && has2(v.x - (1u << rb));
            const bool a1 = nv > 1 && !has2(v.y) && has2(v.y - (1u << rb));
            const bool a2 = nv > 2 && !has2(v.z) && has2(v.z - (1u << rb));
            const bool a3 = nv > 3 && !has2(v.w) && has2(v.w - (1u << rb));
            const bool c0 = a0, c1 = a1, c2 = a2, c3 = a3;
            if (c0 | c1 | c2 | c3) {
              uint32_t idx = atomicAdd(&ctrl[C_NCAND], (uint32_t)c0 + (uint32_t)c1 + (uint32_t)c2 + (uint32_t)c3);
              if (idx + 4u <= pb_cap) {
                const uint16_t y16 = (uint16_t)ysn;
                if (c0) { sb_pos[idx] = v.x; sb_y[idx++] = y16; }
                if (c1) { sb_pos[idx] = v.y; sb_y[idx++] = y16; }
                if (c2) { sb_pos[idx] = v.z; sb_y[idx++] = y16; }
                if (c3) { sb_pos[idx] = v.w; sb_y[idx++] = y16; }
              }
            }
          }
        }
        Step (&sd)[K5_Q] = sdB; k5_u32x4 (&sv)[K5_Q] = svB;
        while (sd[0].n) {
  #pragma unroll
          for (int q = 0; q < K5_Q; q++) {
            const Step& s = sd[q];
            K5_WAIT_OLDEST(sv[q]);
            const uint32_t W = (s.n + 63u) >> 6;
            const uint32_t e0 = k5_lane_times(lane, W);
            const uint32_t mine = min(W, __builtin_elementwise_sub_sat(s.n, e0));
  #ifdef K5_ABL_B
            const uint32_t t0 = 0, t1 = 0, t2 = 0, b3 = ((sv[q].x ^ sv[q].y ^ sv[q].z ^ sv[q].w) == 0x12345678u) << 3;
  #else
            const uint32_t t0 = *K5_LDS((sv[q].x >> sh_a) & tmask4), t1 = *K5_LDS((sv[q].y >> sh_a) & tmask4);
            const uint32_t t2 = *K5_LDS((sv[q].z >> sh_a) & tmask4);
            uint32_t b3 = 0;
            if (W > 3u) b3 = __builtin_amdgcn_ubfe(*K5_LDS((sv[q].w >> sh_a) & tmask4), __builtin_amdgcn_ubfe(sv[q].w, sh_b, 5), 1) << 3;
  #endif
            uint32_t hits = (__builtin_amdgcn_ubfe(t0, __builtin_amdgcn_ubfe(sv[q].x, sh_b, 5), 1) | (__builtin_amdgcn_ubfe(t1, __builtin_amdgcn_ubfe(sv[q].y, sh_b, 5), 1) << 1) |
                             (__builtin_amdgcn_ubfe(t2, __builtin_amdgcn_ubfe(sv[q].z, sh_b, 5), 1) << 2) | b3) &
                            ((1u << mine) - 1u);
            const uint32_t cnt = (uint32_t)__popc(hits);
            if (cnt) {
              const uint32_t ci = atomicAdd(&ctrl[C_NCAND], cnt);
              if (ci + cnt <= pb_cap) {
                uint32_t y16 = s.ysn;
                asm volatile("" : "+v"(y16));
                const uint32_t c1 = ci + (hits & 1u), c2 = ci + (uint32_t)__popc(hits & 3u), c3 = ci + (uint32_t)__popc(hits & 7u);
                if (hits & 1u) { *K5_LDS(pb_pos + (ci << 2)) = sv[q].x; *K5_LDS16(pb_y + (ci << 1)) = (uint16_t)y16; }
                if (hits & 2u) { *K5_LDS(pb_pos + (c1 << 2)) = sv[q].y; *K5_LDS16(pb_y + (c1 << 1)) = (uint16_t)y16; }
                if (hits & 4u) { *K5_LDS(pb_pos + (c2 << 2)) = sv[q].z; *K5_LDS16(pb_y + (c2 << 1)) = (uint16_t)y16; }
                if (hits & 8u) { *K5_LDS(pb_pos + (c3 << 2)) = sv[q].w; *K5_LDS16(pb_y + (c3 << 1)) = (uint16_t)y16; }
              }
            }
            K5_GEN_B(sd[q]); issue(sd[q], sv[q]);
          }
        }
        asm volatile("s_waitcnt vmcnt(0)" ::: "memory");
      }
      }
      __syncthreads();
      if (MULTI) {
        const uint32_t na_raw = ctrl[C_NCAND];
        if (na_raw + 8u > pb_cap) fallback = true;
        const uint32_t na = min(na_raw, pb_cap);
        const unsigned long long below = (1ull << lane) - 1ull;
        for (uint32_t i0 = 0; i0 < na; i0 += nthr) {
          const uint32_t i = i0 + tid;
          const bool live = i < na;
          const uint32_t p = *K5_LDS(pb_pos + ((live ? i : 0u) << 2)), ys = *K5_LDS16(pb_y + ((live ? i : 0u) << 1));
#pragma unroll
          for (int d = 0; d < K5_MAX_ROUNDS; d++) if (d < nrounds) {
            const bool in = live && p - rf_lo[d] <= rf_m1[d];
            const unsigned long long bi = __ballot(in);
            if (bi) {
              uint32_t base = 0;
              if (lane == 0) base = atomicAdd(&ctrl[d == 0 ? C_NCAND0 : C_SPILL + d - 1], (uint32_t)__popcll(bi));
              base = __builtin_amdgcn_readfirstlane(base);
              const uint32_t j = base + (uint32_t)__popcll(bi & below);
              if (in) {
                if (d == 0) { if (j < (uint32_t)cand_cap) { candp[j] = p; candy[j] = (uint16_t)ys; } }
                else if (j < (uint32_t)a.spill_cap) spill_wg[(size_t)(d - 1) * a.spill_cap + j] = make_uint2(p, ys);
              }
            }
          }
        }
        __syncthreads();
        { uint4* h4 = (uint4*)htag; for (int w = tid; w < hclr_q; w += nthr) h4[w] = make_uint4(0, 0, 0, 0); }
        __syncthreads();
      }
    for (int rd = 0; rd < nrounds; rd++) {
      uint32_t c_lo = 0, c_m1 = 0xFFFFFFFFu, f_lo = 0, f_m1 = 0xFFFFFFFFu;
      if (MULTI) {
        const uint64_t rsz64 = 1ull << rb, lo = (uint64_t)rd * a.round_regs * rsz64, hi = rd == nrounds - 1 ? (1ull << 32) : lo + (uint64_t)a.round_regs * rsz64;
        const uint64_t flo = lo >= rsz64 ? lo - rsz64 : 0ull, fhi = hi + rsz64 < (1ull << 32) ? hi + rsz64 : (1ull << 32);
        c_lo = (uint32_t)lo; c_m1 = (uint32_t)(hi - 1ull - lo); f_lo = (uint32_t)flo; f_m1 = (uint32_t)(fhi - 1ull - flo);
      }
      auto in_core = [&](const uint32_t p) -> bool { return !MULTI || p - c_lo <= c_m1; };
      if (MULTI && rd > 0) {
        const uint32_t ns_raw = ctrl[C_SPILL + rd - 1];
        if (ns_raw > (uint32_t)a.spill_cap || ns_raw > (uint32_t)a.cand_limit) fallback = true;
        const uint32_t nsp = min(ns_raw, (uint32_t)min(a.spill_cap, cand_cap));
        const unsigned long long* src = (const unsigned long long*)(spill_wg + (size_t)(rd - 1) * a.spill_cap);
        for (uint32_t i0 = 0; i0 < nsp; i0 += 6u * (uint32_t)nthr) {
          unsigned long long v[6];
#pragma unroll
          for (int k = 0; k < 6; k++) { const uint32_t i = i0 + (uint32_t)k * (uint32_t)nthr + (uint32_t)tid; v[k] = __hip_atomic_load(src + min(i, nsp - 1u), __ATOMIC_RELAXED, __HIP_MEMORY_SCOPE_AGENT); }
#pragma unroll
          for (int k = 0; k < 6; k++) { const uint32_t i = i0 + (uint32_t)k * (uint32_t)nthr + (uint32_t)tid; if (i < nsp) { candp[i] = (uint32_t)v[k]; candy[i] = (uint16_t)(v[k] >> 32); } }
        }
        { uint4* h4 = (uint4*)htag; for (int w = tid; w < hclr_q; w += nthr) h4[w] = make_uint4(0, 0, 0, 0); }
        if (tid == 0) { ctrl[C_NCAND] = ns_raw; ctrl[C_NSTRIP] = 0; ctrl[C_NEDGE] = 0; ctrl[C_NDEFER] = 0; }
      }
      if (rd > 0) __syncthreads();
      K5_STAMP(2);
      const uint32_t nc_raw = ctrl[(MULTI && rd == 0) ? C_NCAND0 : C_NCAND];
      if (nc_raw > (uint32_t)a.cand_limit) fallback = true;
      nc = min(nc_raw, (uint32_t)cand_cap);
      uint32_t* const elist = rec; const uint32_t ecap = 6u * (uint32_t)RC;
      uint32_t* const dlist = elist + (uint32_t)RC; const uint32_t scap = (uint32_t)RC, dcap = ecap - scap;
      auto settle = [&](const uint32_t i, const uint32_t h, const uint32_t off) {
        atomicMax(&hmin[h], 0x10000u - off); atomicMax(&hmax[h], off + 1u);
        candp[i] = (h << 16) | off;
      };
      auto probe_on = [&](const uint32_t i) {
        const uint32_t p = candp[i], r = p >> rb, off = p & rmask;
        const uint32_t h = k5_insert(htag, hmask, hshift, r, true, true);
        if (h != 0xFFFFFFFFu) {
          settle(i, h, off);
          if (off < ovl && r > 0 && k5_insert(htag, hmask, hshift, r - 1u, false) == 0xFFFFFFFFu) ctrl[C_OVERFLOW] = 1u;
        } else ctrl[C_OVERFLOW] = 1u;
      };
      if (!fallback) {
        for (uint32_t i0 = 0; i0 < nc; i0 += nthr) {
          const uint32_t i = i0 + tid;
          const bool live = i < nc;
          const uint32_t p = candp[live ? i : 0u], r = p >> rb, off = p & rmask, r1 = r + 1u;
          const uint32_t h0 = k5_hash(r1, hshift);
          uint32_t prev = 0xFFFFFFFFu;
          if (live) prev = atomicCAS(&htag[h0], 0u, (r1 << 8) | K5_FA | K5_FC);
          const bool hit = live && (prev == 0u || (prev >> 8) == r1);
          if (hit) {
            if (prev != 0u) k5_again(htag, h0, prev, true);
            settle(i, h0, off);
          }
          const bool strip = hit && off < ovl && r > 0, later = live && !hit;
          const unsigned long long bs = __ballot(strip), bd = __ballot(later);
          if (bs | bd) {
            uint32_t sb = 0, db = 0;
            if (lane == 0) { if (bs) sb = atomicAdd(&ctrl[C_NSTRIP], (uint32_t)__popcll(bs)); if (bd) db = atomicAdd(&ctrl[C_NDEFER], (uint32_t)__popcll(bd)); }
            sb = __builtin_amdgcn_readfirstlane(sb); db = __builtin_amdgcn_readfirstlane(db);
            const unsigned long long below = (1ull << lane) - 1ull;
            if (strip) { const uint32_t j = sb + (uint32_t)__popcll(bs & below); if (j < scap) elist[j] = r - 1u; else ctrl[C_OVERFLOW] = 1u; }
            if (later) { const uint32_t j = db + (uint32_t)__popcll(bd & below); if (j < dcap) dlist[j] = i; else probe_on(i); }
          }
        }
      }
      __syncthreads();
      K5_STAMP(10);
      if (!fallback) {
        const uint32_t ns = min(ctrl[C_NSTRIP], scap), nd = min(ctrl[C_NDEFER], dcap);
        for (uint32_t j = tid; j < nd; j += nthr) probe_on(dlist[j]);
        for (uint32_t j = tid; j < ns; j += nthr)
          if (k5_insert(htag, hmask, hshift, elist[j], false) == 0xFFFFFFFFu) ctrl[C_OVERFLOW] = 1u;
      }
      __syncthreads();
      K5_STAMP(3);
      fallback = fallback || rec_over || ctrl[C_OVERFLOW] != 0u;
      if (!fallback) {
        unsigned long long* out = (unsigned long long*)a.out + (size_t)rs * a.out_cap;
        const uint32_t edge = a.D + (uint32_t)max(a.e_max, 0);
        auto emit = [&](const bool memb, const bool keep, const uint32_t p, const uint32_t i) {
          const unsigned long long bm = __ballot(memb), bk = __ballot(keep);
          if (bm) {
            uint32_t base = 0;
            if (lane == 0) { atomicAdd(&ctrl[C_NMEMB], (uint32_t)__popcll(bm)); if (bk) base = atomicAdd(&ctrl[C_NKEEP], (uint32_t)__popcll(bk)); }
            base = __builtin_amdgcn_readfirstlane(base);
            if (keep) {
              const uint32_t slot = base + (uint32_t)__popcll(bk & ((1ull << lane) - 1ull));
              const uint32_t y16 = candy[i];
              if (slot < (uint32_t)a.out_cap) out[slot] = ((unsigned long long)p << 32) | ((unsigned long long)(y16 >> 4) << 16) | (y16 & 15u);
            }
          }
        };
  #ifndef K5_2A_BRANCHY
        {
          const uint32_t do_prune = k_prune, Dv = k_D, emax_on = k_emax_on, emax = k_emax;
          const uint32_t rsz = 1u << rb;
          for (uint32_t i0 = 0; i0 < nc; i0 += nthr) {
            const uint32_t i = i0 + tid;
            const uint32_t valid = i < nc ? 1u : 0u;
            const uint32_t w = candp[valid ? i : 0u], h = w >> 16, off = w & 0xFFFFu;
            const uint32_t town = htag[h], mn = hmin[h], mx = hmax[h];
            const uint32_t r = (town >> 8) - 1u, p = (r << rb) | off;
            const uint32_t is_m = (town >> 1) & 1u , r_pos = r > 0u ? 1u : 0u;
            const uint32_t nb_m = do_prune & (((off < edge ? 1u : 0u) & r_pos) | (off + edge >= rsz ? 1u : 0u)), nb_o = (off < ovl ? 1u : 0u) & r_pos;
            const uint32_t core = in_core(p) ? 1u : 0u;
            const uint32_t nbv = valid & core & (is_m ? nb_m : nb_o);
            const bool nb = nbv != 0u;
            const unsigned long long bn = __ballot(nb);
            if (bn) {
              uint32_t base = 0;
              if (lane == 0) base = atomicAdd(&ctrl[C_NEDGE], (uint32_t)__popcll(bn));
              base = __builtin_amdgcn_readfirstlane(base);
              if (nb) {
                const uint32_t j = base + (uint32_t)__popcll(bn & ((1ull << lane) - 1ull));
                if (j < ecap) elist[j] = i; else ctrl[C_OVERFLOW] = 1u;
              }
            }
            const uint32_t fe = (town >> 4) & 1u , fd = (town >> 3) & 1u ;
            const uint32_t span = (mx - 1u) - (0x10000u - mn);
            const uint32_t iso = fe | (fd & (span <= Dv ? 1u : 0u));
            const uint32_t tight = emax_on & (span <= emax ? 1u : 0u);
            const uint32_t membv = valid & core & is_m & (nbv ^ 1u), keepv = membv & ((iso & (tight ^ 1u)) | (do_prune ^ 1u));
            emit(membv != 0u, keepv != 0u, p, i);
          }
        }
  #else
        for (uint32_t i0 = 0; i0 < nc; i0 += nthr) {
          const uint32_t i = i0 + tid;
          bool memb = false, keep = false; uint32_t p = 0;
          if (i < nc) {
            const uint32_t w = candp[i], h = w >> 16, off = w & 0xFFFFu, town = htag[h], r = (town >> 8) - 1u;
            p = (r << rb) | off;
            const bool is_m = (town & K5_FB) != 0u;
            const bool nb = is_m ? (a.prune && ((off < edge && r > 0) || off + edge >= (1u << rb))) : (off < ovl && r > 0);
            if (nb) {
              const uint32_t j = atomicAdd(&ctrl[C_NEDGE], 1u);
              if (j < ecap) elist[j] = i; else ctrl[C_OVERFLOW] = 1u;
            } else if (is_m) {
              memb = true; keep = true;
              if (a.prune) {
                const uint32_t co = (town & K5_FE) ? 3u : ((town & K5_FD) ? 2u : 1u);
                const uint32_t span = (hmax[h] - 1u) - (0x10000u - hmin[h]);
                keep = co >= 3u || (co == 2u && span <= a.D);
                if (keep && a.e_max >= 0 && span <= (uint32_t)a.e_max) keep = false;
              }
            }
          }
          emit(memb, keep, p, i);
        }
  #endif
        __syncthreads();
        K5_STAMP(11);
        const uint32_t ne = min(ctrl[C_NEDGE], ecap);
        for (uint32_t j0 = 0; j0 < ne; j0 += nthr) {
          const uint32_t j = j0 + tid;
          bool memb = false, keep = false; uint32_t p = 0, i = 0;
          if (j < ne) {
            i = elist[j];
            const uint32_t w = candp[i], hown = w >> 16, off = w & 0xFFFFu, town = htag[hown], r = (town >> 8) - 1u;
            p = (r << rb) | off;
            uint32_t tlf = 0, trt = 0;
            memb = (town & K5_FB) != 0u;
            uint32_t hlf = 0xFFFFFFFFu; bool have_lf = false;
            if (!memb && off < ovl && r > 0) { hlf = k5_find(htag, hmask, hshift, r - 1u, tlf); have_lf = true; memb = (tlf & K5_FB) != 0u; }
            if (memb) {
              keep = true;
              if (a.prune) {
                uint32_t hrt = 0xFFFFFFFFu; trt = 0;
                if (off < edge) { if (!have_lf && r > 0) hlf = k5_find(htag, hmask, hshift, r - 1u, tlf); } else tlf = 0;
                if (off + edge >= (1u << rb)) hrt = k5_find(htag, hmask, hshift, r + 1u, trt);
                const uint32_t co = (town & K5_FE) ? 3u : ((town & K5_FD) ? 2u : 1u);
                const uint32_t omin = 0x10000u - hmin[hown], omax = hmax[hown] - 1u;
                const bool cl = (tlf & K5_FC) != 0u, cr = (trt & K5_FC) != 0u;
                const uint32_t rbase = r << rb;
                keep = co >= 3u || (co == 2u && omax - omin <= a.D);
                uint32_t lmin = 0, lmax = 0, rmin = 0, rmax = 0;
                if (cl) { lmin = 0x10000u - hmin[hlf]; lmax = hmax[hlf] - 1u; }
                if (cr) { rmin = 0x10000u - hmin[hrt]; rmax = hmax[hrt] - 1u; }
                if (!keep && cl) keep = p - (rbase - (1u << rb) + lmax) <= a.D;
                if (!keep && cr) keep = (rbase + (1u << rb) + rmin) - p <= a.D;
                if (keep && a.e_max >= 0) {
                  uint32_t gmin = rbase + omin, gmax = rbase + omax;
                  if (cl) gmin = rbase - (1u << rb) + lmin;
                  if (cr) gmax = rbase + (1u << rb) + rmax;
                  if (gmax - gmin <= (uint32_t)a.e_max) keep = false;
                }
              }
            }
          }
          emit(memb, keep, p, i);
        }
      }
      if (MULTI && rd + 1 < nrounds) { __syncthreads(); if (ctrl[C_OVERFLOW] != 0u) fallback = true; }
    }
    __syncthreads();
    if (ctrl[C_OVERFLOW] != 0u) fallback = true;
    bool prune_only = false;
    if (!fallback && a.prune && ctrl[C_NKEEP] > (uint32_t)a.out_cap) {
      if (!(MULTI && nrounds > 1) && a.raw_out && ctrl[C_NMEMB] <= (uint32_t)a.raw_cap) {
        prune_only = true;
        unsigned long long* raw = (unsigned long long*)a.raw_out + (size_t)rs * a.raw_cap;
        for (int sl = 0; sl < a.n_slabs; sl++) {
        for (uint32_t i0 = 0; i0 < nc; i0 += nthr) {
          const uint32_t i = i0 + tid;
          bool memb = false; uint32_t p = 0;
          if (i < nc) {
            const uint32_t w = candp[i], h = w >> 16, off = w & 0xFFFFu, town = htag[h], r = (town >> 8) - 1u;
            p = (r << rb) | off;
            if ((int)(p >> ix.slab_bits) == sl || (sl == a.n_slabs - 1 && (int)(p >> ix.slab_bits) >= a.n_slabs)) {
              memb = (town & K5_FB) != 0u;
              if (!memb && off < ovl && r > 0) { uint32_t tlf; k5_find(htag, hmask, hshift, r - 1u, tlf); memb = (tlf & K5_FB) != 0u; }
            }
          }
          const unsigned long long bm = __ballot(memb);
          if (bm) {
            uint32_t base = 0;
            if (lane == 0) base = atomicAdd(&ctrl[C_NRAW], (uint32_t)__popcll(bm));
            base = __builtin_amdgcn_readfirstlane(base);
            if (memb) {
              const uint32_t slot = base + (uint32_t)__popcll(bm & ((1ull << lane) - 1ull)), y16 = candy[i];
              if (slot < (uint32_t)a.raw_cap) raw[slot] = ((unsigned long long)p << 32) | ((unsigned long long)(y16 >> 4) << 16) | (y16 & 15u);
            }
          }
        }
        __syncthreads();
        if (tid == 0 && a.surv_seg) { if (sl == 0) a.surv_seg[(size_t)rs * (a.n_slabs + 1)] = 0u; a.surv_seg[(size_t)rs * (a.n_slabs + 1) + sl + 1] = ctrl[C_NRAW]; }
        }
      } else fallback = true;
    }
    K5_STAMP(4);
#ifdef K5_STAMPS
    if (tid == 0) { atomicAdd(&k5_stamps[6], (unsigned long long)nc); if (fallback) atomicAdd(&k5_stamps[7], 1ull); }
#endif
    if (tid == 0) {
      if (fallback) {
        const uint32_t f = atomicAdd(a.fb_cnt, 1u);
        if (f < (uint32_t)a.fb_cap) a.fb_list[f] = (uint32_t)rs; else GS_ADD(a.stats, GS_OVERFLOW_SURV, 1ull);
      } else if (prune_only) {
        const uint32_t nm = ctrl[C_NRAW];
        a.surv_cnt[rs] = nm;
        GS_ADD(a.stats, GS_SURVIVORS, (unsigned long long)nm);
        const uint32_t f = atomicAdd(a.pl_cnt, 1u);
        if (f < (uint32_t)a.pl_cap) a.pl_list[f] = (uint32_t)rs; else GS_ADD(a.stats, GS_OVERFLOW_SURV, 1ull);
      } else {
        const uint32_t nm = ctrl[C_NMEMB], nk = ctrl[C_NKEEP];
        a.surv_cnt[rs] = nm;
        GS_ADD(a.stats, GS_SURVIVORS, (unsigned long long)nm);
        if (a.prune) GS_ADD(a.stats, GS_PRUNED, (unsigned long long)(nm - nk));
        const bool heavy = nk > (uint32_t)a.out_cap;
        if (a.prune) a.out_cnt[rs] = heavy ? 0xFFFFFFFFu : nk;
        if (heavy) {
          const uint32_t hs = atomicAdd(a.heavy_cnt, 1u);
          if (hs < (uint32_t)a.heavy_cap) a.heavy_list[hs] = (uint32_t)rs; else GS_ADD(a.stats, GS_OVERFLOW_SURV, 1ull);
        }
      }
      for (int c = 0; c < C_NLISTS; c++) ctrl[c] = 0;
      *cnl = 0; ctrl[C_NRAW] = 0; ctrl[C_NDEFER] = 0; if (MULTI) ctrl[C_NCAND0] = 0;
      if (MULTI) for (int d = 0; d < K5_MAX_ROUNDS - 1; d++) ctrl[C_SPILL + d] = 0;
    }
    { uint4* t4 = (uint4*)smem; for (int w = tid; w < tab_q; w += nthr) t4[w] = make_uint4(0, 0, 0, 0); }
    K5_STAMP(5);
  }
  for (int d = GM_WAVE / 2; d > 0; d >>= 1) { my_lookups += __shfl_down(my_lookups, d); my_entries += __shfl_down(my_entries, d); }
  if (lane == 0) { GS_ADD(a.stats, GS_LOOKUPS, my_lookups); GS_ADD(a.stats, GS_ENTRIES, my_entries); }
}
```

Baseline: 3.473 million.

## Replace precomputed strip index with inline overlap-strip detection in lookup kernel

Removes the derived per-seed strip position lists (sdir/spos) and their separate marking and candidate passes. The kernel now spots overlap-strip entries inline while streaming the main position lists, marking and testing the previous region in the same loop. This drops the extra strip directory loads, the session-time derivation with its scan, and the srec LDS records, and it reuses the freed LDS to enlarge xrec. In exchange it adds per-element compare and bit-loop work in the hot loops, and the enable condition for the v5 path moves from checking whether strips exist to checking slab count.

```diff
diff --git a/shrimp_amd/csrc/gm_common.h b/shrimp_amd/csrc/gm_common.h
--- a/shrimp_amd/csrc/gm_common.h
+++ b/shrimp_amd/csrc/gm_common.h
@@ -24,8 +24,6 @@
   const uint32_t* dir;
   const uint32_t* pos;
   const uint32_t* bkt;
-  const uint32_t* sdir;
-  const uint32_t* spos;
   uint32_t n_pos;
 };
 
diff --git a/shrimp_amd/csrc/gm_host.hip b/shrimp_amd/csrc/gm_host.hip
--- a/shrimp_amd/csrc/gm_host.hip
+++ b/shrimp_amd/csrc/gm_host.hip
@@ -108,7 +108,6 @@
   for (int i = 0; i < n_seeds; i++) {
     d.seed[i].mask = seeds[i].mask; d.seed[i].span = seeds[i].span; d.seed[i].weight = seeds[i].weight;
     d.seed[i].dir = seeds[i].d_dir; d.seed[i].pos = seeds[i].d_pos; d.seed[i].bkt = seeds[i].d_bkt; d.seed[i].n_pos = seeds[i].n_pos;
-    d.seed[i].sdir = strips_ready ? seeds[i].d_sdir : nullptr; d.seed[i].spos = strips_ready ? seeds[i].d_spos : nullptr;
   }
   return d;
 }
@@ -273,8 +272,7 @@
   if (!ix) return;
   (void)hipSetDevice(ix->device);
   (void)hipFree(ix->d_genome); (void)hipFree(ix->d_genome_cs); (void)hipFree(ix->d_contig_off); (void)hipFree(ix->d_contig_rna);
-  for (int i = 0; i < ix->n_seeds; i++) { (void)hipFree(ix->seeds[i].d_dir); (void)hipFree(ix->seeds[i].d_pos); (void)hipFree(ix->seeds[i].d_bkt);
-                                           (void)hipFree(ix->seeds[i].d_sdir); (void)hipFree(ix->seeds[i].d_spos); }
+  for (int i = 0; i < ix->n_seeds; i++) { (void)hipFree(ix->seeds[i].d_dir); (void)hipFree(ix->seeds[i].d_pos); (void)hipFree(ix->seeds[i].d_bkt); }
   delete ix;
 }
 extern "C" uint32_t gm_index_list_cutoff(const gm_index_t* ix) { return ix->list_cutoff; }
@@ -282,8 +280,7 @@
 extern "C" int gm_index_has_buckets(const gm_index_t* ix) { return ix->seeds[0].d_bkt != nullptr; }
 extern "C" uint64_t gm_index_bytes(const gm_index_t* ix) {
   uint64_t b = ix->genome_words * 4 * (ix->d_genome_cs ? 2 : 1);
-  for (int i = 0; i < ix->n_seeds; i++) b += (ix->seeds[i].dir_words + (uint64_t)ix->seeds[i].n_pos + (ix->seeds[i].d_bkt ? (16ull << ix->seeds[i].kbits) : 0ull) +
-                                            (ix->seeds[i].d_sdir ? (1ull << ix->seeds[i].kbits) + 1 + ix->seeds[i].n_spos : 0ull)) * 4;
+  for (int i = 0; i < ix->n_seeds; i++) b += (ix->seeds[i].dir_words + (uint64_t)ix->seeds[i].n_pos + (ix->seeds[i].d_bkt ? (16ull << ix->seeds[i].kbits) : 0ull)) * 4;
   return b;
 }
 extern "C" int gm_index_get_list(const gm_index_t* ix, int sn, uint32_t mapidx, uint32_t* len, uint32_t* positions, uint32_t cap) {
@@ -653,10 +650,6 @@
   GM_HIP_S(hipHostMalloc((void**)&s->h_pin, (16 + 1024) * 4, hipHostMallocDefault));
   memset(s->h_pin, 0, (16 + 1024) * 4);
   { const int rc = gm_index_derive_rna(const_cast<gm_index*>(ix), s->stream); if (rc) { gm_session_free(s); return rc; } }
-  if ((ix->n_slabs > 1 || gm_tune("GM_K1_V5")) && !gm_tune("GM_NO_V5") && ix->params.region_bits >= 9 && ix->params.region_bits <= 16) {
-    const int rc = gm_index_derive_strips(const_cast<gm_index*>(ix), s->stream);
-    if (rc) { gm_session_free(s); return rc; }
-  }
   *out = s;
   return GM_OK;
 #undef GM_HIP_S
diff --git a/shrimp_amd/csrc/gm_internal.h b/shrimp_amd/csrc/gm_internal.h
--- a/shrimp_amd/csrc/gm_internal.h
+++ b/shrimp_amd/csrc/gm_internal.h
@@ -5,7 +5,6 @@
   uint64_t mask = 0; int span = 0, weight = 0;
   int kbits = 0;
   uint32_t* d_dir = nullptr; uint32_t* d_pos = nullptr; uint32_t* d_bkt = nullptr;
-  uint32_t* d_sdir = nullptr; uint32_t* d_spos = nullptr; uint32_t n_spos = 0;
   uint32_t n_pos = 0; uint64_t dir_words = 0;
   std::string text;
 };
@@ -25,7 +24,6 @@
   int slab_bits = 29, n_slabs = 1;
   gm_params_t params;
   uint32_t list_cutoff = 0;
-  bool strips_ready = false;
   double fasta_to_bitfield_s = 0, fasta_total_s = 0;
   GmIndexDev dev_view() const;
 };
@@ -85,7 +83,6 @@
                      unsigned long long* d_stats, hipStream_t stream, GmK1Scratch* K, uint32_t* d_surv_seg = nullptr,
                      const GmFusePrune* fuse = nullptr);
 int gm_index_derive_rna(GmIndexHost* ix, hipStream_t stream);
-int gm_index_derive_strips(GmIndexHost* ix, hipStream_t stream);
 int gm_lookup5_launch(const GmIndexDev& ix, const uint32_t* d_reads, int n_reads, int read_len, int read_words, int max_n_kmers, int NL,
                       uint64_t* d_out, uint32_t* d_out_cnt, int out_cap, uint32_t* d_surv_cnt, int prune, uint32_t D, int e_max,
                       uint32_t* d_heavy_list, uint32_t* d_heavy_cnt, int heavy_cap, unsigned long long* d_stats, hipStream_t stream, GmK1Scratch* K,
diff --git a/shrimp_amd/csrc/gm_lookup5.hip b/shrimp_amd/csrc/gm_lookup5.hip
--- a/shrimp_amd/csrc/gm_lookup5.hip
+++ b/shrimp_amd/csrc/gm_lookup5.hip
@@ -1,9 +1,7 @@
 #include <algorithm>
 #include <cmath>
-#include <mutex>
 #include "gm_common.h"
 #include "gm_internal.h"
-#include <rocprim/device/device_scan.hpp>
 
 typedef uint32_t k5_u32x4 __attribute__((ext_vector_type(4), aligned(4)));
 typedef __attribute__((address_space(3))) uint32_t k5_lds_u32;
@@ -83,85 +81,13 @@
 #undef K5_KERNEL_MULTI
 #undef K5_KERNEL_LSWC
 
-__device__ __forceinline__ bool k5_strip(uint32_t p, int rb, uint32_t ovl) { return (p & ((1u << rb) - 1u)) < ovl && (p >> rb) > 0u; }
-
-__global__ void __launch_bounds__(256) k_strip_count(const uint32_t* __restrict__ pos, uint32_t n_pos, int rb, uint32_t ovl, uint32_t* __restrict__ grp_cnt, uint32_t n_groups) {
-  const uint32_t lane = threadIdx.x & 63u;
-  uint64_t g = ((uint64_t)blockIdx.x * blockDim.x + threadIdx.x) >> 6;
-  const uint64_t stride = ((uint64_t)gridDim.x * blockDim.x) >> 6;
-  for (; g < n_groups; g += stride) {
-    const uint64_t i = g * 64 + lane;
-    const bool f = i < n_pos && k5_strip(pos[i], rb, ovl);
-    const unsigned long long b = __ballot(f);
-    if (lane == 0) grp_cnt[g] = (uint32_t)__popcll(b);
-  }
-}
-__global__ void __launch_bounds__(256) k_strip_scatter(const uint32_t* __restrict__ pos, uint32_t n_pos, int rb, uint32_t ovl, const uint32_t* __restrict__ grp_rank,
-                                                       uint32_t n_groups, uint32_t* __restrict__ spos) {
-  const uint32_t lane = threadIdx.x & 63u;
-  uint64_t g = ((uint64_t)blockIdx.x * blockDim.x + threadIdx.x) >> 6;
-  const uint64_t stride = ((uint64_t)gridDim.x * blockDim.x) >> 6;
-  for (; g < n_groups; g += stride) {
-    const uint64_t i = g * 64 + lane;
-    const uint32_t p = i < n_pos ? pos[i] : 0u;
-    const bool f = i < n_pos && k5_strip(p, rb, ovl);
-    const unsigned long long b = __ballot(f);
-    if (f) spos[grp_rank[g] + (uint32_t)__popcll(b & ((1ull << lane) - 1ull))] = p;
-  }
-}
-__global__ void __launch_bounds__(256) k_strip_dir(const uint32_t* __restrict__ dir, const uint32_t* __restrict__ pos, uint32_t n_pos, uint64_t K, int S, int rb, uint32_t ovl,
-                                                   const uint32_t* __restrict__ grp_rank, uint32_t* __restrict__ sdir) {
-  uint64_t k = (uint64_t)blockIdx.x * blockDim.x + threadIdx.x;
-  const uint64_t stride = (uint64_t)gridDim.x * blockDim.x;
-  for (; k <= K; k += stride) {
-    const uint32_t i = dir[k * (uint64_t)S];
-    uint32_t r = grp_rank[i >> 6];
-    for (uint32_t q = i & ~63u; q < i; q++) r += k5_strip(pos[q], rb, ovl) ? 1u : 0u;
-    sdir[k] = r;
-  }
-}
-
-static std::mutex g_strip_mutex;
-int gm_index_derive_strips(GmIndexHost* ix, hipStream_t stream) {
-  std::lock_guard<std::mutex> lock(g_strip_mutex);
-  if (ix->strips_ready) return GM_OK;
-  const int rb = ix->params.region_bits; const uint32_t ovl = (uint32_t)ix->params.region_overlap;
-  for (int sn = 0; sn < ix->n_seeds; sn++) {
-    GmSeedHost& sd = ix->seeds[sn];
-    const uint64_t K = 1ull << sd.kbits;
-    const uint32_t n_groups = (uint32_t)(((uint64_t)sd.n_pos + 63) / 64) + 1u;
-    uint32_t *d_cnt = nullptr, *d_rank = nullptr; void* tmp = nullptr; size_t tmp_bytes = 0;
-    GM_HIP(hipMalloc(&d_cnt, (size_t)n_groups * 4)); GM_HIP(hipMalloc(&d_rank, (size_t)n_groups * 4));
-    hipLaunchKernelGGL(k_strip_count, dim3(256 * 16), dim3(256), 0, stream, sd.d_pos, sd.n_pos, rb, ovl, d_cnt, n_groups);
-    hipError_t e = rocprim::exclusive_scan(nullptr, tmp_bytes, d_cnt, d_rank, 0u, (size_t)n_groups, rocprim::plus<uint32_t>(), stream);
-    if (e != hipSuccess) { gm_set_error("exclusive_scan size query: %s", hipGetErrorString(e)); return GM_E_NODEVICE; }
-    GM_HIP(hipMalloc(&tmp, tmp_bytes ? tmp_bytes : 16));
-    e = rocprim::exclusive_scan(tmp, tmp_bytes, d_cnt, d_rank, 0u, (size_t)n_groups, rocprim::plus<uint32_t>(), stream);
-    if (e != hipSuccess) { gm_set_error("exclusive_scan: %s", hipGetErrorString(e)); return GM_E_NODEVICE; }
-    uint32_t total = 0;
-    GM_HIP(hipMemcpyAsync(&total, d_rank + (n_groups - 1), 4, hipMemcpyDeviceToHost, stream));
-    GM_HIP(hipStreamSynchronize(stream));
-    sd.n_spos = total;
-    GM_HIP(hipMalloc(&sd.d_spos, ((size_t)total + 64) * 4));
-    GM_HIP(hipMemsetAsync(sd.d_spos, 0xff, ((size_t)total + 64) * 4, stream));
-    GM_HIP(hipMalloc(&sd.d_sdir, (size_t)(K + 1 + 16) * 4));
-    hipLaunchKernelGGL(k_strip_scatter, dim3(256 * 16), dim3(256), 0, stream, sd.d_pos, sd.n_pos, rb, ovl, d_rank, n_groups, sd.d_spos);
-    hipLaunchKernelGGL(k_strip_dir, dim3(256 * 16), dim3(256), 0, stream, sd.d_dir, sd.d_pos, sd.n_pos, K, ix->n_slabs, rb, ovl, d_rank, sd.d_sdir);
-    GM_HIP(hipGetLastError());
-    GM_HIP(hipStreamSynchronize(stream));
-    (void)hipFree(d_cnt); (void)hipFree(d_rank); (void)hipFree(tmp);
-  }
-  ix->strips_ready = true;
-  return GM_OK;
-}
-
 int gm_lookup5_launch(const GmIndexDev& ix, const uint32_t* d_reads, int n_reads, int read_len, int read_words, int max_n_kmers, int NL,
                       uint64_t* d_out, uint32_t* d_out_cnt, int out_cap, uint32_t* d_surv_cnt, int prune, uint32_t D, int e_max,
                       uint32_t* d_heavy_list, uint32_t* d_heavy_cnt, int heavy_cap, unsigned long long* d_stats, hipStream_t stream, GmK1Scratch* K,
                       uint64_t* d_raw, int raw_cap, uint32_t* d_surv_seg) {
   int dev = 0; if (hipGetDevice(&dev) != hipSuccess) return 0;
-  if (!ix.seed[0].sdir || ix.region_bits < 9 || ix.region_bits > 16 || NL <= 0) return 0;
   const bool forced = gm_tune("GM_K1_V5") != nullptr;
+  if ((ix.n_slabs < 2 && !forced) || ix.region_bits < 9 || ix.region_bits > 16 || NL <= 0) return 0;
   double entries = 0;
   for (int sn = 0; sn < ix.n_seeds; sn++) {
     const double lists = std::max(0, read_len - ix.seed[sn].span + 1 - ix.colour);
@@ -169,7 +95,7 @@
   }
   if (!forced && entries < 8000.0) return 0;
   const size_t budget = 160 * 1024 - 512;
-  const size_t fixed0 = (size_t)24 * NL + 2 * (size_t)((read_len + 15) & ~15) + C_WORDS * 4 + GM_MAX_SEEDS * 32;
+  const size_t fixed0 = (size_t)24 * NL + 2 * (size_t)((read_len + 15) & ~15) + C_WORDS * 4 + GM_MAX_SEEDS * 16;
   const size_t full_tables = (size_t)(4u << 15) + (size_t)(4u << 12);
   int xrec = read_len > 128 ? 16 : 64;
   if (fixed0 + 24 * (size_t)xrec + full_tables > budget && fixed0 + 24 * 16 + full_tables <= budget) xrec = (int)((budget - full_tables - fixed0) / 24);
@@ -238,7 +164,7 @@
   if (const char* e = gm_tune("GM_K5_GRID")) grid = std::max(1, std::min(2 * n_reads, atoi(e)));
   K5Args a;
   a.reads = d_reads; a.n_reads = n_reads; a.read_len = read_len; a.read_words = read_words; a.max_n_kmers = max_n_kmers; a.NL = NL;
-  a.lsw = lsw; a.ltw = ltw; a.cand_cap = cand_cap; a.hbits = hbits; a.cand_limit = cand_limit; a.xrec = xrec; a.rounds = rounds; a.round_regs = round_regs;
+  a.lsw = lsw; a.ltw = ltw; a.cand_cap = cand_cap; a.hbits = hbits; a.cand_limit = cand_limit; a.xrec = (int)(24 * (size_t)(NL + xrec) / 16) - NL; a.rounds = rounds; a.round_regs = round_regs;
   a.out = d_out; a.out_cnt = d_out_cnt; a.out_cap = out_cap; a.surv_cnt = d_surv_cnt; a.prune = prune; a.D = D; a.e_max = e_max;
   a.heavy_list = d_heavy_list; a.heavy_cnt = d_heavy_cnt; a.heavy_cap = heavy_cap; a.stats = d_stats;
   a.fb_list = K->k5_fb; a.fb_cnt = fb_cnt_p; a.fb_cap = fb_cap;
diff --git a/shrimp_amd/csrc/gm_lookup5_kernel.inc b/shrimp_amd/csrc/gm_lookup5_kernel.inc
--- a/shrimp_amd/csrc/gm_lookup5_kernel.inc
+++ b/shrimp_amd/csrc/gm_lookup5_kernel.inc
@@ -27,19 +27,16 @@
   uint32_t* hmax = hmin + (1u << hbits);
   uint32_t* rec = seen + (1u << lsw);
   const int RC = a.NL + a.xrec;
-  uint32_t* srec = rec + 4 * RC;
-  uint8_t* codes = (uint8_t*)(srec + 2 * RC);
+  uint8_t* codes = (uint8_t*)(rec + 4 * RC);
   uint32_t* ctrl = (uint32_t*)(codes + 2 * ((a.read_len + 15) & ~15));
-  const uint32_t smask4 = wmask << 2, tmask4 = tmask << 2, swb = 4u << ltw;
+  const uint32_t smask4 = wmask << 2, tmask4 = tmask << 2, swb = 4u << ltw, rsz = 1u << rb;
   const int sh_a = rb - 2, sh_b = rb + lsw;
   const uint32_t hmask = (1u << hbits) - 1u; const int hshift = 32 - hbits;
   const uint32_t pb_cap = MULTI ? (2u << hbits) : (uint32_t)cand_cap;
   const uint32_t pb_pos = MULTI ? swb + (4u << hbits) : swb, pb_y = pb_pos + 4u * pb_cap;
-  uint32_t* const sb_pos = MULTI ? htag : candp; uint16_t* const sb_y = (uint16_t*)(sb_pos + pb_cap);
   const int hclr_q = (int)(3u << hbits) >> 2;
   const int tab_q = (int)(((1u << ltw) + (1u << lsw)) >> 2);
   const uint32_t* __restrict__ pos0 = ix.seed[0].pos;
-  const uint32_t* __restrict__ spos0 = ix.seed[0].spos;
   unsigned long long my_lookups = 0, my_entries = 0;
   uint32_t k_prune = __builtin_amdgcn_readfirstlane(a.prune != 0 ? 1u : 0u), k_D = __builtin_amdgcn_readfirstlane(a.D);
   uint32_t k_emax_on = __builtin_amdgcn_readfirstlane(a.e_max >= 0 ? 1u : 0u), k_emax = __builtin_amdgcn_readfirstlane((uint32_t)max(a.e_max, 0));
@@ -49,19 +46,26 @@
   if (tid < C_WORDS) ctrl[tid] = 0;
 
   auto bloom_mask = [&](const uint32_t t) -> uint32_t { return (1u << (t & 31u)) | (2u << ((t + (((t >> 5) & 3u) << 2)) & 31u)); };
-  auto mark = [&](const uint32_t p) {
-    const uint32_t av = p >> sh_a, t = p >> sh_b, m1 = 1u << (t & 31u), m = BLOOM ? bloom_mask(t) : m1;
+  auto strip_slots = [&](const k5_u32x4& v) -> uint32_t {
+    return ((v.x & rmask) < ovl ? 1u : 0u) | ((v.y & rmask) < ovl ? 2u : 0u) | ((v.z & rmask) < ovl ? 4u : 0u) | ((v.w & rmask) < ovl ? 8u : 0u);
+  };
+  auto slot_of = [&](const k5_u32x4& v, const uint32_t k) -> uint32_t { const uint32_t lo = (k & 1u) ? v.y : v.x, hi = (k & 1u) ? v.w : v.z; return (k & 2u) ? hi : lo; };
+  auto mark_before = [&](const uint32_t p) {
+    const uint32_t q = p - rsz, av = q >> sh_a, t = q >> sh_b, m1 = p >= rsz ? 1u << (t & 31u) : 0u, m = BLOOM ? (p >= rsz ? bloom_mask(t) : 0u) : m1;
     const uint32_t old = K5_LDS_OR(swb + (av & smask4), m);
-    if ((old & m) == m) K5_LDS_OR(av & tmask4, m1);
+    K5_LDS_OR(av & tmask4, BLOOM ? ((old & m) == m ? m1 : 0u) : (old & m));
   };
-  auto has2 = [&](const uint32_t p) -> bool { return (*K5_LDS((p >> sh_a) & tmask4) >> ((p >> sh_b) & 31u)) & 1u; };
+  auto has2_before = [&](const uint32_t p) -> uint32_t {
+    const uint32_t q = p - rsz;
+    return p >= rsz ? (*K5_LDS((q >> sh_a) & tmask4) >> ((q >> sh_b) & 31u)) & 1u : 0u;
+  };
 
 #ifdef K5_STAMPS
   unsigned long long t_prev = __builtin_amdgcn_s_memtime();
 #endif
   const bool ahead = a.NL <= nthr;
   const uint32_t cpad = (uint32_t)((a.read_len + 15) & ~15);
-  uint32_t pf_b = 0, pf_e = 0, pf_sb = 0, pf_se = 0; bool pf_ok = false;
+  uint32_t pf_b = 0, pf_e = 0; bool pf_ok = false;
   auto fill_codes = [&](const int r, uint8_t* cb) {
     if (r >= 2 * a.n_reads) return;
     const uint32_t* rw = a.reads + (size_t)(r >> 1) * a.read_words;
@@ -70,9 +74,8 @@
   uint32_t* stab = ctrl + C_WORDS;
   if (tid < ix.n_seeds) {
     const GmSeedDev& sd = ix.seed[tid];
-    const uint64_t d = (uint64_t)(uintptr_t)sd.dir, sdp = (uint64_t)(uintptr_t)sd.sdir, po = (uint64_t)(sd.pos - pos0), so = (uint64_t)(sd.spos - spos0);
-    *(uint4*)&stab[8 * tid] = make_uint4((uint32_t)d, (uint32_t)(d >> 32), (uint32_t)sdp, (uint32_t)(sdp >> 32));
-    *(uint4*)&stab[8 * tid + 4] = make_uint4((uint32_t)po, (uint32_t)(po >> 32), (uint32_t)so, (uint32_t)(so >> 32));
+    const uint64_t d = (uint64_t)(uintptr_t)sd.dir, po = (uint64_t)(sd.pos - pos0);
+    *(uint4*)&stab[4 * tid] = make_uint4((uint32_t)d, (uint32_t)(d >> 32), (uint32_t)po, (uint32_t)(po >> 32));
   }
   int k_sn = 0, k_i = 0, k_span = 0; uint64_t k_mask = 0; bool k_ok = false;
   const int k_stride = 1, k_slot = tid;
@@ -84,25 +87,18 @@
     if (!k_ok) { k_span = 0; k_mask = 0; }
   }
   uint32_t* cnl_w = nullptr;
-  auto strip_of = [&](const int j0, uint32_t& slen) -> const uint32_t* {
-    const uint2 sr = *(const uint2*)&srec[2 * j0];
-    const uint4 st = *(const uint4*)&stab[8 * (rec[4 * j0 + 3] & 15u) + 4];
-    slen = sr.y;
-    return spos0 + ((((uint64_t)st.w << 32) | st.z) + sr.x);
-  };
-  auto put_records = [&](const uint64_t la, const uint32_t len, const uint32_t ysn, const uint32_t sb, const uint32_t slen) {
+  auto put_records = [&](const uint64_t la, const uint32_t len, const uint32_t ysn) {
     const uint32_t nch = (len + 255u) >> 8;
     const uint32_t j = atomicAdd(cnl_w, nch);
     for (uint32_t c = 0; c < nch && j + c < (uint32_t)RC; c++) {
       const uint64_t ca = la + ((uint64_t)c << 10);
       *(uint4*)&rec[4 * (j + c)] = make_uint4((uint32_t)ca, (uint32_t)(ca >> 32), min(256u, len - (c << 8)), ((ysn >> 12) & 0xFFF0u) | (ysn & 0xFu));
-      *(uint2*)&srec[2 * (j + c)] = c ? make_uint2(0u, 0u) : make_uint2(sb, slen);
     }
   };
-  auto put_list = [&](const uint32_t b, const uint32_t n, const uint32_t sb, const uint32_t sn) {
-    const uint4 so = *(const uint4*)&stab[8 * k_sn + 4];
+  auto put_list = [&](const uint32_t b, const uint32_t n) {
+    const uint2 so = *(const uint2*)&stab[4 * k_sn + 2];
     const uint64_t ptr = (((uint64_t)so.y << 32) | so.x) + b;
-    put_records((uint64_t)(uintptr_t)(pos0 + ptr), n, ((uint32_t)k_i << 16) | (uint32_t)k_sn, sb, sn);
+    put_records((uint64_t)(uintptr_t)(pos0 + ptr), n, ((uint32_t)k_i << 16) | (uint32_t)k_sn);
   };
   auto kmer_ahead = [&](const int r, const uint8_t* cb) {
     pf_ok = k_ok && r < 2 * a.n_reads;
@@ -118,11 +114,10 @@
       }
     } else if (pf_ok) mapidx = gm_mapidx(ix, k_mask, k_span, cb + k_i);
     if (!pf_ok) mapidx = 0;
-    const uint4 sp = *(const uint4*)&stab[8 * k_sn];
+    const uint2 sp = *(const uint2*)&stab[4 * k_sn];
     typedef const uint32_t __attribute__((address_space(1)))* k5_gptr;
     const k5_gptr dir = (k5_gptr)(((uint64_t)sp.y << 32) | sp.x) + (size_t)mapidx * (uint32_t)S;
-    const k5_gptr sdir = (k5_gptr)(((uint64_t)sp.w << 32) | sp.z) + mapidx;
-    pf_b = dir[0]; pf_e = dir[S]; pf_sb = sdir[0]; pf_se = sdir[1];
+    pf_b = dir[0]; pf_e = dir[S];
   };
   uint32_t rf_lo[K5_MAX_ROUNDS], rf_m1[K5_MAX_ROUNDS];
 #pragma unroll
@@ -140,11 +135,11 @@
     cnl_w = cnl;
     if (ahead) {
       fill_codes(rs + (int)gridDim.x, codes + (uint32_t)((it + 1) & 1) * cpad);
-      const uint32_t b = pf_b, e = pf_e, sb = pf_sb, se = pf_se;
-      if ((b ^ e ^ sb ^ se) == 0x9E3779B9u && e - b == 0x7F4A7C15u) ctrl[C_SINK] = 1u;
+      const uint32_t b = pf_b, e = pf_e;
+      if ((b ^ e) == 0x9E3779B9u && e - b == 0x7F4A7C15u) ctrl[C_SINK] = 1u;
       const bool has_list = pf_ok && e != b && e - b <= ix.list_cutoff;
       if (pf_ok) my_lookups++;
-      if (has_list) { my_entries += (e - b); put_list(b, e - b, sb, se - sb); }
+      if (has_list) { my_entries += (e - b); put_list(b, e - b); }
       __syncthreads();
       K5_STAMP(8);
       kmer_ahead(rs + (int)gridDim.x, codes + (uint32_t)((it + 1) & 1) * cpad);
@@ -163,9 +158,8 @@
       my_lookups++;
       const uint32_t b = dir[0], e = dir[S];
       if (e == b || e - b > ix.list_cutoff) continue;
-      const uint32_t sb = ix.seed[sn].sdir[mapidx], se = ix.seed[sn].sdir[mapidx + 1];
       my_entries += (e - b);
-      put_records((uint64_t)(uintptr_t)(ix.seed[sn].pos + b), e - b, ((uint32_t)i << 16) | (uint32_t)sn, sb, se - sb);
+      put_records((uint64_t)(uintptr_t)(ix.seed[sn].pos + b), e - b, ((uint32_t)i << 16) | (uint32_t)sn);
     }
     __syncthreads();
     }
@@ -237,19 +231,6 @@
     for (int a_rep = 0; a_rep < 2; a_rep++)
 #endif
     {
-#ifndef K5_ABL_NOSTRIP
-      for (int j0 = tid >> 2; j0 < nl; j0 += nthr >> 2) {
-        uint32_t slen; const uint32_t* sp = strip_of(j0, slen);
-        for (uint32_t e = (uint32_t)(tid & 3) * 4u; e < slen; e += 16u) {
-          const k5_u32x4 v = *(const k5_u32x4*)(sp + e);
-          const uint32_t nv = min(4u, slen - e);
-          mark(v.x - (1u << rb));
-          if (nv > 1) mark(v.y - (1u << rb));
-          if (nv > 2) mark(v.z - (1u << rb));
-          if (nv > 3) mark(v.w - (1u << rb));
-        }
-      }
-#endif
       gen_reset();
       Step sd[K5_Q]; k5_u32x4 sv[K5_Q];
 #pragma unroll
@@ -286,6 +267,8 @@
             K5_TWICE(a2, o2 & m2);
             if (W > 3) K5_TWICE(a3, o3 & m3);
             }
+            uint32_t ss = strip_slots(sv[q]) & ((1u << W) - 1u);
+            if (ss) do { mark_before(slot_of(sv[q], (uint32_t)__builtin_ctz(ss))); ss &= ss - 1u; } while (ss);
 #endif
           }
           gen(sd[q]); issue(sd[q], sv[q]);
@@ -307,35 +290,6 @@
       {
       if (!MULTI) { uint4* h4 = (uint4*)htag; for (int w = tid; w < hclr_q; w += nthr) h4[w] = make_uint4(0, 0, 0, 0); }
       {
-        for (int j0 = tid >> 2; j0 <
-#ifdef K5_ABL_NOSTRIP
-             0
-#else
-             nl
-#endif
-             ; j0 += nthr >> 2) {
-          uint32_t slen; const uint32_t* sp = strip_of(j0, slen);
-          const uint32_t ysn = rec[4 * j0 + 3];
-          for (uint32_t e = (uint32_t)(tid & 3) * 4u; e < slen; e += 16u) {
-            const k5_u32x4 v = *(const k5_u32x4*)(sp + e);
-            const uint32_t nv = min(4u, slen - e);
-            const bool a0 = !has2(v.x) && has2(v.x - (1u << rb));
-            const bool a1 = nv > 1 && !has2(v.y) && has2(v.y - (1u << rb));
-            const bool a2 = nv > 2 && !has2(v.z) && has2(v.z - (1u << rb));
-            const bool a3 = nv > 3 && !has2(v.w) && has2(v.w - (1u << rb));
-            const bool c0 = a0, c1 = a1, c2 = a2, c3 = a3;
-            if (c0 | c1 | c2 | c3) {
-              uint32_t idx = atomicAdd(&ctrl[C_NCAND], (uint32_t)c0 + (uint32_t)c1 + (uint32_t)c2 + (uint32_t)c3);
-              if (idx + 4u <= pb_cap) {
-                const uint16_t y16 = (uint16_t)ysn;
-                if (c0) { sb_pos[idx] = v.x; sb_y[idx++] = y16; }
-                if (c1) { sb_pos[idx] = v.y; sb_y[idx++] = y16; }
-                if (c2) { sb_pos[idx] = v.z; sb_y[idx++] = y16; }
-                if (c3) { sb_pos[idx] = v.w; sb_y[idx++] = y16; }
-              }
-            }
-          }
-        }
         Step (&sd)[K5_Q] = sdB; k5_u32x4 (&sv)[K5_Q] = svB;
         while (sd[0].n) {
   #pragma unroll
@@ -356,6 +310,8 @@
             uint32_t hits = (__builtin_amdgcn_ubfe(t0, __builtin_amdgcn_ubfe(sv[q].x, sh_b, 5), 1) | (__builtin_amdgcn_ubfe(t1, __builtin_amdgcn_ubfe(sv[q].y, sh_b, 5), 1) << 1) |
                              (__builtin_amdgcn_ubfe(t2, __builtin_amdgcn_ubfe(sv[q].z, sh_b, 5), 1) << 2) | b3) &
                             ((1u << mine) - 1u);
+            uint32_t ss = strip_slots(sv[q]) & ((1u << mine) - 1u) & ~hits;
+            if (ss) do { const uint32_t k = (uint32_t)__builtin_ctz(ss); hits |= has2_before(slot_of(sv[q], k)) << k; ss &= ss - 1u; } while (ss);
             const uint32_t cnt = (uint32_t)__popc(hits);
             if (cnt) {
               const uint32_t ci = atomicAdd(&ctrl[C_NCAND], cnt);
@@ -433,8 +389,8 @@
       const uint32_t nc_raw = ctrl[(MULTI && rd == 0) ? C_NCAND0 : C_NCAND];
       if (nc_raw > (uint32_t)a.cand_limit) fallback = true;
       nc = min(nc_raw, (uint32_t)cand_cap);
-      uint32_t* const elist = rec; const uint32_t ecap = 6u * (uint32_t)RC;
-      uint32_t* const dlist = elist + (uint32_t)RC; const uint32_t scap = (uint32_t)RC, dcap = ecap - scap;
+      uint32_t* const elist = rec; const uint32_t ecap = 4u * (uint32_t)RC;
+      const uint32_t scap = 2u * (uint32_t)RC / 3u, dcap = ecap - scap; uint32_t* const dlist = elist + scap;
       auto settle = [&](const uint32_t i, const uint32_t h, const uint32_t off) {
         atomicMax(&hmin[h], 0x10000u - off); atomicMax(&hmax[h], off + 1u);
         candp[i] = (h << 16) | off;
```

New measurement: 3.158 million. 9.0% lower.
